# yjtang249/MIPSFusion

Measured on AMD Instinct MI355X. Metric: rays*samples/s per GPU, full optimisation iteration (fwd + bwd + pose+map Adam), 4096 rays x 64 samples, 640x480 RGB-D, higher is better.
Workload: dtype f32; decoder products as 3 x bf16 pieces of each fp32 operand, 6 bf16 MFMAs per product, fp32 accumulate; 1 GPU; BASELINE config 2: FastCaMo-synth apartment_2, 1 active submap per GPU, 4096 rays x 64 samples, hash grid 2^19 x 16 x 2, 620x460 synthetic RGB-D; rays=4096, samples_per_ray=64, hash_size=19, parallelism=single gpu

## Files before the change

### include/mipsf_compact.h

```cpp
#ifndef MIPSF_COMPACT_H
#define MIPSF_COMPACT_H

#include "mipsf.h"

#ifdef __cplusplus
extern "C" {
#endif

#define MIPSF_LIVE_HEADER 16u
#define MIPSF_LIVE_PAD 0xffffffffu
int mipsf_decoder_live_compact(const float* dout, uint32_t M, uint32_t* live_list, float* dfeat, float* dx, int feat_layout,
                               void* stream);

int mipsf_hashgrid_dx_from_jac_list(const float* jac, const float* dout, float* dx, const uint32_t* live_list, uint32_t M,
                                    const mipsf_grid_meta* meta_host, int layout, void* stream);

#ifdef __cplusplus
}
#endif
#endif
```

### mipsfusion_amd/_lib.py

```python
from __future__ import annotations

import ctypes as C
import os
from typing import Optional

import torch

_HERE = os.path.dirname(os.path.abspath(__file__))
LIB_PATH = os.environ.get("MIPSF_LIB") or os.path.join(_HERE, "libmipsf_hip.so")
MAX_LEVELS = 32
FEAT_AOS, FEAT_LEVEL_MAJOR = 0, 1
PREC = {"f32": 0, "f16x3": 1, "f16": 2, "bf16x3": 3, "bf16x6": 4}


class GridMeta(C.Structure):
    _fields_ = [("n_levels", C.c_uint32), ("n_features", C.c_uint32), ("log2_hashmap_size", C.c_uint32),
                ("base_resolution", C.c_uint32), ("per_level_scale", C.c_float),
                ("log2_per_level_scale", C.c_float), ("n_params", C.c_uint32),
                ("offsets", C.c_uint32 * (MAX_LEVELS + 1)), ("resolutions", C.c_uint32 * MAX_LEVELS),
                ("scales", C.c_float * MAX_LEVELS)]


class DecoderWeights(C.Structure):
    _fields_ = [(n, C.c_void_p) for n in ("w_pts0", "b_pts0", "w_pts2", "b_pts2", "w_rgb0", "b_rgb0",
# ... 17 lines not shown
        a = cls()
        a.struct_size = C.sizeof(cls)
        for k, v in kw.items():
            setattr(a, k, v)
        return a
    cls.new = staticmethod(new)
    return cls


_VP, _CU, _CI = C.c_void_p, C.c_uint32, C.c_int
HashgridBwdArgs = _args("HashgridBwdArgs", [("M", _CU), ("x", _VP), ("params", _VP), ("dout", _VP), ("dparams", _VP), ("dx", _VP),
                                            ("scratch", _VP), ("counters", _VP), ("meta", C.POINTER(GridMeta)),
                                            ("feat_layout", _CI), ("flags", _CU)])
DecoderFwd16Args = _args("DecoderFwd16Args", [("M", _CU), ("packed16", _VP), ("feat", _VP), ("x", _VP), ("out", _VP), ("saved", _VP),
                                              ("tile_live_clear", _VP), ("feat_layout", _CI), ("precision", _CI),
                                              ("sdf_only", _CI), ("lean_record", _CI), ("packed16_floats", _CU)])
DecoderChain16Args = _args("DecoderChain16Args", [("M", _CU), ("packed16", _VP), ("x", _VP), ("out", _VP), ("dout", _VP),
                                                  ("saved", _VP), ("dfeat", _VP), ("dx", _VP), ("dact", _VP), ("tile_live", _VP),
                                                  ("feat_layout", _CI), ("flags", _CI), ("packed16_floats", _CU),
                                                  ("live_list", _VP)])
DecoderWgrad16Args = _args("DecoderWgrad16Args", [("M", _CU), ("packed16", _VP), ("feat", _VP), ("x", _VP), ("saved", _VP),
                                                  ("dact", _VP), ("tile_live", _VP), ("grads", C.POINTER(DecoderGrads)),
                                                  ("partial", _VP), ("feat_layout", _CI), ("arithmetic", _CI), ("flags", _CU),
                                                  ("packed16_floats", _CU), ("live_list", _VP)])
RenderFwdArgs = _args("RenderFwdArgs", [("N", _CU), ("S", _CU), ("raw", _VP), ("z_vals", _VP), ("target_rgb", _VP), ("target_d", _VP),
                                        ("counts", _VP), ("cfg", C.POINTER(RenderCfg)), ("rgb", _VP), ("depth", _VP),
                                        ("depth_var", _VP), ("disp", _VP), ("acc", _VP), ("weights", _VP), ("losses", _VP),
                                        ("partial", _VP), ("loss_weights", _VP), ("loss_total", _VP), ("ticket", _VP),
                                        ("sums", _VP), ("draw", _VP)])
RenderBwdArgs = _args("RenderBwdArgs", [("N", _CU), ("S", _CU), ("N_norm", _CU), ("raw", _VP), ("z_vals", _VP), ("target_rgb", _VP),
                                        ("target_d", _VP), ("counts", _VP), ("losses", _VP), ("cfg", C.POINTER(RenderCfg)),
                                        ("g_losses", _VP), ("g_total", _VP), ("loss_weights", _VP), ("g_rgb", _VP),
                                        ("g_depth", _VP), ("draw", _VP), ("flags", _CU)])
RENDER_BWD_KEEP_IF_UNIT = 1

(SIZE_HASHGRID_BWD_SCRATCH, SIZE_HASHGRID_COUNTER_WORDS, SIZE_DECODER_PACKED, SIZE_DECODER_SAVED, SIZE_DECODER_DACT,
 SIZE_DECODER_WGRAD_PARTIAL, SIZE_DECODER_PACKED16, SIZE_DECODER_TILE_WORDS, SIZE_RENDER_PARTIAL, SIZE_PLACE_POSE_SCRATCH,
 SIZE_POSE_RAYS_SCRATCH, SIZE_HASHGRID_DET_SCRATCH, SIZE_DECODER_LIVE_LIST) = range(1, 14)
LIVE_HEADER, LIVE_PAD = 16, 0xFFFFFFFF

HG_DPARAMS_ZERO, HG_ROUTED, HG_DETERMINISTIC = 1, 2, 4
HG_DET_PIECE = 512
HG_DET_MAX_ITEMS = 1 << 31
TILE_ORDER_MAX_M = 1 << 27
WGRAD_LEAN_DACT, WGRAD_DETERMINISTIC = 1, 2


ADAM_MAX_TENSORS = 16


class AdamTensors(C.Structure):
    _fields_ = [("count", C.c_uint32), ("param", C.c_void_p * ADAM_MAX_TENSORS), ("grad", C.c_void_p * ADAM_MAX_TENSORS),
                ("exp_avg", C.c_void_p * ADAM_MAX_TENSORS), ("exp_avg_sq", C.c_void_p * ADAM_MAX_TENSORS),
                ("numel", C.c_uint64 * ADAM_MAX_TENSORS)]


ADAM_MAX_GROUPS = 8
ADAM_SMALL_MAX_NUMEL = 16384


class AdamSmall(C.Structure):
    _fields_ = [("n_groups", C.c_uint32), ("n_tensors", C.c_uint32),
                ("step_dev", C.c_void_p * ADAM_MAX_GROUPS), ("hyper_dev", C.c_void_p * ADAM_MAX_GROUPS),
                ("lr", C.c_float * ADAM_MAX_GROUPS), ("beta1", C.c_float * ADAM_MAX_GROUPS),
                ("beta2", C.c_float * ADAM_MAX_GROUPS), ("eps", C.c_float * ADAM_MAX_GROUPS),
                ("weight_decay", C.c_float * ADAM_MAX_GROUPS),
                ("param", C.c_void_p * ADAM_MAX_TENSORS), ("grad", C.c_void_p * ADAM_MAX_TENSORS),
                ("exp_avg", C.c_void_p * ADAM_MAX_TENSORS), ("exp_avg_sq", C.c_void_p * ADAM_MAX_TENSORS),
                ("numel", C.c_uint32 * ADAM_MAX_TENSORS), ("group_of", C.c_uint32 * ADAM_MAX_TENSORS)]


_P = C.c_void_p
_U32, _U64, _I, _F, _D = C.c_uint32, C.c_uint64, C.c_int, C.c_float, C.c_double

SIGNATURES = {
    "mipsf_last_error": (C.c_char_p, []),
    "mipsf_abi_version": (_I, []),
    "mipsf_device_cu_count": (_I, []),
    "mipsf_buffer_size": (_U64, [_I, _U32, _U32, _U32, C.POINTER(GridMeta)]),
    "mipsf_hashgrid_meta_init": (_I, [C.POINTER(GridMeta), _U32, _U32, _U32, _U32, _D]),
    "mipsf_hashgrid_fwd": (_I, [_P, _P, _P, _P, _U32, C.POINTER(GridMeta), _I, _P]),
    "mipsf_hashgrid_dx_from_jac": (_I, [_P, _P, _P, _P, _U32, C.POINTER(GridMeta), _I, _P]),
    "mipsf_hashgrid_bwd": (_I, [C.POINTER(HashgridBwdArgs), _P]),
    "mipsf_hashgrid_route": (_I, [_P, _P, _U32, C.POINTER(GridMeta), _P]),
    "mipsf_hashgrid_indices": (_I, [_P, _P, _U32, C.POINTER(GridMeta), _P]),
    "mipsf_freq_fwd": (_I, [_P, _P, _U32, _U32, _U32, _P]),
    "mipsf_freq_bwd": (_I, [_P, _P, _P, _U32, _U32, _U32, _P]),
    "mipsf_decoder_pack": (_I, [C.POINTER(DecoderWeights), _P, _P]),
    "mipsf_decoder_pack_host": (_I, [C.POINTER(DecoderWeights), _P]),
    "mipsf_decoder_fwd": (_I, [_P, _P, _I, _P, _P, _I, _P, _P, _U32, _P]),
    "mipsf_decoder_fwd_sdf": (_I, [_P, _P, _I, _P, _P, _I, _P, _U32, _P]),
    "mipsf_decoder_bwd": (_I, [_P, _P, _I, _P, _P, _I, _P, _P, _P, _P, _P, _P, C.POINTER(DecoderGrads), _P, _P,
                               _U32, _P]),
    "mipsf_decoder_bwd_chain": (_I, [_P, _I, _P, _I, _P, _P, _P, _P, _P, _P, _P, _U32, _P]),
    "mipsf_decoder_wgrad": (_I, [_P, _I, _P, _P, _I, _P, _P, C.POINTER(DecoderGrads), _P, _I, _U32, _P]),
    "mipsf_decoder_pack16": (_I, [C.POINTER(DecoderWeights), _P, _I, _P]),
    "mipsf_decoder_fwd16": (_I, [C.POINTER(DecoderFwd16Args), _P]),
    "mipsf_decoder_bwd_chain16": (_I, [C.POINTER(DecoderChain16Args), _P]),
    "mipsf_decoder_wgrad16": (_I, [C.POINTER(DecoderWgrad16Args), _P]),
    "mipsf_sample_rays": (_I, [_P, _P, _P, _P, _P, _P, _P, C.POINTER(RenderCfg), _P, _P, _P, _U32, _P]),
    "mipsf_normalise_points": (_I, [_P, C.POINTER(RenderCfg), _P, _U32, _P]),
    "mipsf_render_fwd": (_I, [C.POINTER(RenderFwdArgs), _P]),
    "mipsf_loss_finalize_sums": (_I, [_P, C.POINTER(RenderCfg), _U32, _U32, _P, _P, _P, _P]),
    "mipsf_render_bwd": (_I, [C.POINTER(RenderBwdArgs), _P]),
    "mipsf_gather_pose_place_fwd": (_I, [_P, _U64, _P, _P, _P, _P, _U32, _U32, _P, _P, _P, _P, _P, C.POINTER(RenderCfg), _P, _P,
                                         _P, _P, _P, _P, _U32, _P]),
    "mipsf_place_pose_bwd": (_I, [_P, _P, C.POINTER(RenderCfg), _P, _U32, _U32, _P, _P, _P, _P, _P, _U32, _U32, _I, _P]),
    "mipsf_rays_bwd": (_I, [_P, _P, C.POINTER(RenderCfg), _P, _P, _U32, _U32, _P]),
    "mipsf_normalise_bwd": (_I, [_P, C.POINTER(RenderCfg), _P, _U32, _P]),
    "mipsf_pose_rays_fwd": (_I, [_P, _U64, _P, _P, _P, _P, _U32, _U32, _P, _P, _P, _P, _P, _P, _U32, _P]),
    "mipsf_pose_handover": (_I, [_P, _I, _P, _P, _P]),
    "mipsf_pose_rays_bwd": (_I, [_P, _P, _P, _U32, _U32, _P, _P, _P, _P, _P, _U32, _I, _P]),
    "mipsf_adam_step": (_I, [_P, _P, _P, _P, _U64, _F, _F, _F, _F, _F, _U32, _P, _I, _P]),
    "mipsf_adam_advance_n": (_I, [_P, _P, _P, _P, _P, _U32, _P]),
    "mipsf_adam_step_multi": (_I, [C.POINTER(AdamTensors), _F, _F, _F, _F, _F, _U32, _P, _I, _P]),
    "mipsf_adam_step_small": (_I, [C.POINTER(AdamSmall), _I, _P]),
    "mipsf_adam_step_all": (_I, [C.POINTER(AdamSmall), _I, _P, _P]),
    "mipsf_ro_fitness": (_I, [_P, _U32, _P, _F, _P, _U32, _U32, _P]),
    "mipsf_ro_fitness_sdf": (_I, [_P, _P, _F, _P, _U32, _U32, _I, _P]),
    "mipsf_ro_particles": (_I, [_P, _P, _P, _P, C.POINTER(RenderCfg), _P, _P, _U32, _U32, _I, _P]),
    "mipsf_ro_update": (_I, [_P, _P, _P, _F, _F, _U32, _P]),
    "mipsf_gather_rays": (_I, [_P, _U64, _P, _U32, _P, _P, _P, _P, _P]),
}


SIZE_MCUBES_OFFSET_WORDS, SIZE_MCUBES_WELD_SLOTS, SIZE_MCUBES_WELD_WORDS = 20, 21, 22
MCUBES_BLOCK_CELLS = 4096
McubesArgs = _args("McubesArgs", [("X", _CU), ("Y", _CU), ("Z", _CU), ("isovalue", C.c_float), ("truncation", C.c_float),
                                  ("volume", _VP), ("cases", _VP), ("block_offsets", _VP), ("soup", _VP), ("cell_ids", _VP),
                                  ("capacity_tris", _CU)])
McubesWeldArgs = _args("McubesWeldArgs", [("T", _CU), ("soup", _VP), ("scratch", _VP), ("vertices", _VP), ("faces", _VP),
                                          ("counts", _VP), ("max_rounds", _CU)])
COMPACT_SIGNATURES = {
    "mipsf_decoder_live_compact": (_I, [_P, _U32, _P, _P, _P, _I, _P]),
    "mipsf_hashgrid_dx_from_jac_list": (_I, [_P, _P, _P, _P, _U32, C.POINTER(GridMeta), _I, _P]),
}

MESH_SIGNATURES = {
    "mipsf_mcubes_count": (_I, [C.POINTER(McubesArgs), _P]),
    "mipsf_mcubes_emit": (_I, [C.POINTER(McubesArgs), _P]),
    "mipsf_mcubes_weld": (_I, [C.POINTER(McubesWeldArgs), _P]),
}


FUSE_KF_FLOATS = 16
FUSE_IN_BOX, FUSE_SEEN = 1, 2


class FusePoints(C.Structure):
    _fields_ = [("points", _VP), ("ticks", _VP * 3), ("dims", _CU * 3), ("lo", _CU * 3), ("size", _CU * 3), ("first", _CU), ("n", _CU)]


class FuseCamera(C.Structure):
    _fields_ = [("fx", C.c_float), ("fy", C.c_float), ("cx", C.c_float), ("cy", C.c_float), ("W", C.c_float), ("H", C.c_float),
                ("edge", C.c_float), ("k", _CU), ("keyframes", _VP)]


FuseVisibilityArgs = _args("FuseVisibilityArgs", [("pts", FusePoints), ("cam", FuseCamera), ("seen", _VP)])
FuseLocalArgs = _args("FuseLocalArgs", [("pts", FusePoints), ("w2l", C.c_float * 12), ("sub", C.c_double * 3), ("div", C.c_double * 3),
                                        ("out", _VP)])
FuseAccumulateArgs = _args("FuseAccumulateArgs", [("pts", FusePoints), ("cam", FuseCamera), ("rows", _VP), ("n_rows", _CU),
                                                  ("channels", _CU), ("sigmoid", _CU), ("values", _VP), ("entropy", _VP),
                                                  ("value_stride", _CU), ("entropy_stride", _CU), ("use_obb", _CU),
                                                  ("obb_centre", C.c_double * 3), ("obb_axes", C.c_double * 9),
                                                  ("obb_half", C.c_double * 3), ("centroid", C.c_float * 3), ("sigma", C.c_float),
                                                  ("gauss_k", C.c_float), ("num", _VP), ("den", _VP), ("flags", _VP)])
FuseFinalizeArgs = _args("FuseFinalizeArgs", [("n", _CU), ("channels", _CU), ("num", _VP), ("den", _VP), ("flags", _VP), ("out", _VP),
                                              ("volume", _VP)])
FuseLabelArgs = _args("FuseLabelArgs", [("F", _CU), ("E", _CU), ("pairs", _VP), ("labels", _VP), ("counts", _VP), ("max_rounds", _CU),
                                        ("resume", _CU)])
FUSE_SIGNATURES = {
    "mipsf_fuse_visibility": (_I, [C.POINTER(FuseVisibilityArgs), _P]),
    "mipsf_fuse_local_points": (_I, [C.POINTER(FuseLocalArgs), _P]),
    "mipsf_fuse_accumulate": (_I, [C.POINTER(FuseAccumulateArgs), _P]),
    "mipsf_fuse_finalize": (_I, [C.POINTER(FuseFinalizeArgs), _P]),
    "mipsf_fuse_label_components": (_I, [C.POINTER(FuseLabelArgs), _P]),
}


ICP_KNN = 30
ICP_RESULT_DOUBLES = 20
ICP_MAX_POINTS, ICP_MAX_CELLS = 1 << 27, 1 << 26
ICP_WS_CLOUD, ICP_WS_GRID, ICP_WS_REGISTER = 1, 2, 3
IcpCloudArgs = _args("IcpCloudArgs", [("n", _CU), ("k", _CU), ("rows_per_owner", _CU), ("rows", _VP), ("owner", _VP), ("poses", _VP),
                                      ("points", _VP), ("count", _VP), ("workspace", _VP)])
IcpBinArgs = _args("IcpBinArgs", [("n", _CU), ("max_cells", _CU), ("points", _VP), ("min_edge", C.c_double), ("grid", _VP)])
IcpNearestArgs = _args("IcpNearestArgs", [("n_source", _CU), ("n_target", _CU), ("max_cells", _CU), ("source", _VP), ("grid", _VP),
                                          ("max_dist", C.c_double), ("partner", _VP), ("d2", _VP)])
IcpNormalsArgs = _args("IcpNormalsArgs", [("n", _CU), ("max_cells", _CU), ("points", _VP), ("grid", _VP), ("normals", _VP),
                                          ("neighbours", _VP)])
IcpRegisterArgs = _args("IcpRegisterArgs", [("n_source", _CU), ("n_target", _CU), ("max_cells", _CU), ("max_iteration", _CU),
                                            ("source", _VP), ("grid", _VP), ("target_normals", _VP), ("max_dist", C.c_double),
                                            ("relative_fitness", C.c_double), ("relative_rmse", C.c_double), ("result", _VP),
                                            ("partner", _VP), ("workspace", _VP)])
ICP_SIGNATURES = {
    "mipsf_icp_workspace_bytes": (_U64, [_I, _U32, _U32]),
    "mipsf_icp_cloud": (_I, [C.POINTER(IcpCloudArgs), _P]),
    "mipsf_icp_bin": (_I, [C.POINTER(IcpBinArgs), _P]),
    "mipsf_icp_nearest": (_I, [C.POINTER(IcpNearestArgs), _P]),
    "mipsf_icp_normals": (_I, [C.POINTER(IcpNormalsArgs), _P]),
    "mipsf_icp_register": (_I, [C.POINTER(IcpRegisterArgs), _P]),
}


POSEGRAPH_MAX_NODES, POSEGRAPH_MAX_EDGES, POSEGRAPH_LDS_NODES, POSEGRAPH_RESULT_DOUBLES = 64, 1024, 20, 8
POSEGRAPH_FACTORISATION_FAILED, POSEGRAPH_NAN_QUALITY, POSEGRAPH_BAD_EDGE = 1, 2, 4
PosegraphArgs = _args("PosegraphArgs", [("n_nodes", _CU), ("n_edges", _CU), ("input_f64", _CU), ("anchors", _VP), ("edges", _VP),
                                        ("observations", _VP), ("weights", _VP), ("steps", _CU), ("patience", _CU),
                                        ("max_rejects", _CU), ("reserved", _CU), ("decreasing", C.c_double), ("radius", C.c_double),
                                        ("min_diag", C.c_double), ("anchors_out", _VP), ("anchors_out32", _VP), ("result", _VP),
                                        ("workspace", _VP)])
POSEGRAPH_SIGNATURES = {
    "mipsf_posegraph_workspace_bytes": (_U64, [_U32, _U32]),
    "mipsf_posegraph_optimize": (_I, [C.POINTER(PosegraphArgs), _P]),
}


SUBMAP_MAX_BOXES, SUBMAP_MAX_TOP_KF, SUBMAP_HEADER_WORDS, SUBMAP_BOX_WORDS, SUBMAP_WORKSPACE_BYTES = 64, 10, 16, 12, 8192
# ... 69 lines not shown
    "mipsf_raster_workspace_bytes": (_U64, [_I, _U32, _U32, _U32, _U32]),
    "mipsf_raster_depth": (_I, [C.POINTER(RasterDepthArgs), _P]),
    "mipsf_raster_l1": (_I, [C.POINTER(RasterL1Args), _P]),
    "mipsf_raster_visible": (_I, [C.POINTER(RasterVisibleArgs), _P]),
}


TSDF_MAX_VOXELS, TSDF_MAX_SIDE, TSDF_VIEW_CHUNK, TSDF_BRICK = 0x7FFFFFFF, 8192, 256, (8, 8, 16)
TSDF_NO_CULL = 1
TSDF_MAX_BRICKS = 0xFFFFFF
TSDF_RECORD_WORDS = 2
TsdfIntegrateArgs = _args("TsdfIntegrateArgs", [("X", _CU), ("Y", _CU), ("Z", _CU), ("n", _CU), ("H", _CU), ("W", _CU), ("flags", _CU),
                                                ("fx", C.c_double), ("fy", C.c_double), ("cx", C.c_double), ("cy", C.c_double),
                                                ("trunc", C.c_double), ("depth_max", C.c_double), ("max_weight", C.c_double),
                                                ("ticks", _VP * 3), ("depth", _VP), ("rgb", _VP), ("poses", _VP), ("tsdf", _VP),
                                                ("weight", _VP), ("color", _VP), ("record", _VP)])
TsdfSampleArgs = _args("TsdfSampleArgs", [("X", _CU), ("Y", _CU), ("Z", _CU), ("m", _CU), ("reserved", _CU), ("points", _VP),
                                          ("weight", _VP), ("color", _VP), ("out", _VP)])
TSDF_SIGNATURES = {
    "mipsf_tsdf_integrate": (_I, [C.POINTER(TsdfIntegrateArgs), _P]),
    "mipsf_tsdf_sample": (_I, [C.POINTER(TsdfSampleArgs), _P]),
}


TRACK_MAX_SAMPLES, TRACK_TILE, TRACK_RESULT_DOUBLES, TRACK_MAX_ITERATION, TRACK_MAX_VIEWS = 0x100000, 16, 20, 1000, 65535
TRACK_NO_SKIP = 1
TRACK_WS_RAYCAST, TRACK_WS_REGISTER = 1, 2
TRACK_RECORD_WORDS = 2
TrackRaycastArgs = _args("TrackRaycastArgs", [("X", _CU), ("Y", _CU), ("Z", _CU), ("n", _CU), ("H", _CU), ("W", _CU), ("flags", _CU),
                                              ("origin", C.c_double * 3), ("voxel", C.c_double), ("trunc", C.c_double),
                                              ("fx", C.c_double), ("fy", C.c_double), ("cx", C.c_double), ("cy", C.c_double),
                                              ("near", C.c_double), ("far", C.c_double), ("step", C.c_double), ("min_weight", C.c_double),
                                              ("tsdf", _VP), ("weight", _VP), ("color", _VP), ("poses", _VP), ("depth", _VP),
                                              ("normals", _VP), ("color_out", _VP), ("record", _VP), ("workspace", _VP)])
TrackRegisterArgs = _args("TrackRegisterArgs", [("H", _CU), ("W", _CU), ("max_iteration", _CU),
                                                ("fx", C.c_double), ("fy", C.c_double), ("cx", C.c_double), ("cy", C.c_double),
                                                ("depth_max", C.c_double), ("max_dist", C.c_double), ("relative_fitness", C.c_double),
                                                ("relative_rmse", C.c_double), ("model_depth", _VP), ("model_normals", _VP),
                                                ("pose_ref", _VP), ("live", _VP), ("pose_init", _VP), ("result", _VP), ("pose_out", _VP),
                                                ("partner", _VP), ("workspace", _VP)])
TRACK_SIGNATURES = {
    "mipsf_track_workspace_bytes": (_U64, [_I, _U32, _U32, _U32]),
    "mipsf_track_raycast": (_I, [C.POINTER(TrackRaycastArgs), _P]),
    "mipsf_track_register": (_I, [C.POINTER(TrackRegisterArgs), _P]),
}


IMAGE_F32, IMAGE_F64 = 0, 1
IMAGE_WINDOW, IMAGE_TILE_H, IMAGE_TILE_W, IMAGE_MAX_CHANNELS, IMAGE_MAX_SIDE = 11, 16, 32, 4, 8192
IMAGE_MAX_PLANES, IMAGE_MAX_VALUES, IMAGE_ERROR_MAX_BLOCKS = 65535, 0x7FFFFFFF, 256
IMAGE_WS_ERROR, IMAGE_WS_SSIM = 1, 2
IMAGE_ERROR_RECORD_BYTES, IMAGE_SSIM_RECORD_BYTES = 32, 32


class ImageErrorRecord(C.Structure):
    _fields_ = [("sum_sq", C.c_double), ("sum_abs", C.c_double), ("max_abs", C.c_double), ("count", C.c_uint64)]


class ImageSsimRecord(C.Structure):
    _fields_ = [("sum_ssim", C.c_double), ("sum_cs", C.c_double), ("count", C.c_uint64), ("reserved", C.c_uint64)]


ImageErrorArgs = _args("ImageErrorArgs", [("n", _CU), ("H", _CU), ("W", _CU), ("C", _CU), ("dtype", _CU), ("a", _VP), ("b", _VP),
                                          ("records", _VP), ("workspace", _VP)])
ImageSsimArgs = _args("ImageSsimArgs", [("n", _CU), ("H", _CU), ("W", _CU), ("C", _CU), ("dtype", _CU), ("window", C.c_double * 11),
                                        ("C1", C.c_double), ("C2", C.c_double), ("a", _VP), ("b", _VP), ("records", _VP),
                                        ("workspace", _VP)])
ImagePool2Args = _args("ImagePool2Args", [("n", _CU), ("H", _CU), ("W", _CU), ("C", _CU), ("dtype", _CU), ("in_", _VP), ("out", _VP)])
IMAGE_SIGNATURES = {
    "mipsf_image_workspace_bytes": (_U64, [_I, _U32, _U32, _U32, _U32]),
    "mipsf_image_error": (_I, [C.POINTER(ImageErrorArgs), _P]),
    "mipsf_image_ssim": (_I, [C.POINTER(ImageSsimArgs), _P]),
    "mipsf_image_pool2": (_I, [C.POINTER(ImagePool2Args), _P]),
}


def buffer_size(which: int, n: int = 0, a: int = 0, b: int = 0, meta=None) -> int:
    v = lib().mipsf_buffer_size(which, n, a, b, C.byref(meta) if meta is not None else None)
    if v == 0xFFFFFFFFFFFFFFFF:
        raise RuntimeError((lib().mipsf_last_error() or b"mipsf_buffer_size: bad query").decode())
    return int(v)


_lib: Optional[C.CDLL] = None


def lib() -> C.CDLL:
    global _lib
    if _lib is None:
        if not os.path.exists(LIB_PATH):
            raise RuntimeError(
                f"{LIB_PATH} is missing: build it with `python -c 'import __graft_entry__ as g; g.build()'` "
                "(or `make -C mipsfusion_amd/csrc`). There is no CPU fallback.")
        handle = C.CDLL(LIB_PATH)
        for name, (res, args) in list(SIGNATURES.items()) + (list(MESH_SIGNATURES.items())
                                       + list(FUSE_SIGNATURES.items()) + list(ICP_SIGNATURES.items())
                                       + list(COMPACT_SIGNATURES.items()) + list(POSEGRAPH_SIGNATURES.items())
                                       + list(SUBMAP_SIGNATURES.items()) + list(EVAL_SIGNATURES.items())
                                       + list(RASTER_SIGNATURES.items()) + list(TSDF_SIGNATURES.items())
                                       + list(IMAGE_SIGNATURES.items()) + list(TRACK_SIGNATURES.items())):
            fn = getattr(handle, name)
            fn.restype = res
            fn.argtypes = args
        if handle.mipsf_abi_version() != 2:
            raise RuntimeError("libmipsf_hip.so ABI version mismatch")
        _lib = handle
    return _lib


KEPT_BLOCK_CACHES = []


def check(rc: int, what: str = "") -> None:
    if rc != 0:
        msg = lib().mipsf_last_error().decode(errors="replace")
        for cache in KEPT_BLOCK_CACHES:
            cache.clear()
        raise RuntimeError(f"libmipsf_hip {what} failed (code {rc}): {msg}")


def stream_ptr() -> int:
    return torch._C._cuda_getCurrentRawStream(torch._C._cuda_getDevice())


def dptr(t: Optional[torch.Tensor], dtype=torch.float32) -> Optional[int]:
    if t is None:
        return None
    if not t.is_cuda:
        raise RuntimeError("mipsfusion_amd operators need GPU tensors (no CPU fallback exists)")
    if t.device.index != torch._C._cuda_getDevice():
        raise RuntimeError(f"tensor lives on cuda:{t.device.index} but the current device is "
                           f"cuda:{torch._C._cuda_getDevice()}; wrap the call in torch.cuda.device(tensor.device)")
    if t.dtype != dtype:
        raise RuntimeError(f"expected {dtype}, got {t.dtype}")
    if not t.is_contiguous():
        raise RuntimeError("tensor must be contiguous")
    return t.data_ptr()


def make_grid_meta(n_levels=16, n_features=2, log2_hashmap_size=19, base_resolution=16,
                   per_level_scale=2.0) -> GridMeta:
    m = GridMeta()
    check(lib().mipsf_hashgrid_meta_init(C.byref(m), n_levels, n_features, log2_hashmap_size, base_resolution,
                                         float(per_level_scale)), "hashgrid_meta_init")
    return m
```

### mipsfusion_amd/csrc/hashgrid.hip

```cpp
#include "common.h"
#include "decoder_layout.h"

namespace mipsf {

constexpr uint32_t P1 = 2654435761u;
constexpr uint32_t P2 = 805459861u;
constexpr int HG_BLOCK = 256;

struct Cell {
    uint32_t c[3];
    float f[3];
};

__device__ __forceinline__ Cell locate(const float* __restrict__ x, uint32_t i, float scale) {
    Cell r;
#pragma unroll
    for (int d = 0; d < 3; ++d) {
        const float pos = fmaf(scale, x[3 * (size_t)i + d], 0.5f);
        const float fl = floorf(pos);
        r.c[d] = (uint32_t)(int)fl;
        r.f[d] = pos - fl;
    }
    return r;
}
// ... 7 lines not shown
            idx -= size;
            if (idx >= size) idx %= size;
        }
        return idx;
    }
    const uint32_t h = cx ^ (cy * P1) ^ (cz * P2);
    return MODE == 1 ? (h & (size - 1u)) : (h % size);
}

__host__ __device__ inline bool level_is_hashed(uint32_t res, uint32_t size) {
    uint64_t stride = 1;
    for (int d = 0; d < 3; ++d) {
        if (stride > size) break;
        stride *= res;
        stride &= 0xFFFFFFFFull;
    }
    return size < stride;
}

__device__ __forceinline__ int decode_level(uint32_t n_levels, uint32_t nchunk, uint32_t& chunk) {
    const uint32_t b = blockIdx.x;
    const uint32_t xcd = b & 7u;
    const uint32_t j = b >> 3;
    const uint32_t slot = j / nchunk;
    chunk = j - slot * nchunk;
    const uint32_t nslots = (n_levels + 7u) / 8u;
    return (int)(xcd + 8u * (nslots - 1u - slot));
}

template <int MODE>
__device__ __forceinline__ void corner_indices_m(const Cell& cell, uint32_t res, uint32_t size, uint32_t idx[8]) {
#pragma unroll
    for (int c = 0; c < 8; ++c) {
        idx[c] = corner_index<MODE>(cell.c[0] + (c & 1), cell.c[1] + ((c >> 1) & 1), cell.c[2] + ((c >> 2) & 1),
                                    res, size);
    }
}

__device__ __forceinline__ int level_mode(uint32_t res, uint32_t size) {
    if (!level_is_hashed(res, size)) return 0;
    return (size & (size - 1u)) == 0u ? 1 : 2;
}

__device__ __forceinline__ void corner_indices(int mode, const Cell& cell, uint32_t res, uint32_t size,
                                               uint32_t idx[8]) {
    if (mode == 0) corner_indices_m<0>(cell, res, size, idx);
    else if (mode == 1) corner_indices_m<1>(cell, res, size, idx);
    else corner_indices_m<2>(cell, res, size, idx);
}

__device__ __forceinline__ void corner_weights(const Cell& cell, float w[8]) {
#pragma unroll
    for (int c = 0; c < 8; ++c) {
        float t = (c & 1) ? cell.f[0] : 1.0f - cell.f[0];
        t = t * ((c & 2) ? cell.f[1] : 1.0f - cell.f[1]);
        t = t * ((c & 4) ? cell.f[2] : 1.0f - cell.f[2]);
        w[c] = t;
    }
}

template <int LAYOUT>
__device__ __forceinline__ size_t feat_index(uint32_t i, uint32_t level, uint32_t M, uint32_t L) {
    return LAYOUT == MIPSF_FEAT_AOS ? ((size_t)i * L + level) * 2 : ((size_t)level * M + i) * 2;
}

__device__ __forceinline__ void level_jacobian(const Cell& cell, const float2 (&v)[8], float scale, int d, float& s0,
                                               float& s1) {
    s0 = 0.f, s1 = 0.f;
#pragma unroll
    for (int sub = 0; sub < 4; ++sub) {
        const int d0 = d == 0 ? 1 : 0;
        const int d1 = d == 2 ? 1 : 2;
        const int b0 = sub & 1, b1 = (sub >> 1) & 1;
        float wgt = scale;
        wgt = wgt * (b0 ? cell.f[d0] : 1.0f - cell.f[d0]);
        wgt = wgt * (b1 ? cell.f[d1] : 1.0f - cell.f[d1]);
        const int left = (b0 << d0) | (b1 << d1);
        const int right = left | (1 << d);
        s0 = s0 + wgt * (v[right].x - v[left].x);
        s1 = s1 + wgt * (v[right].y - v[left].y);
    }
}

template <int LAYOUT, bool JAC>
__global__ __launch_bounds__(HG_BLOCK) void hashgrid_fwd_kernel(const float* __restrict__ x,
                                                                const float2* __restrict__ table,
                                                                float* __restrict__ out, float* __restrict__ jac,
                                                                uint32_t M, GridLevels g, uint32_t nchunk) {
    uint32_t chunk;
    const int level = decode_level(g.n_levels, nchunk, chunk);
    if (level >= (int)g.n_levels) return;
    const uint32_t i = chunk * HG_BLOCK + threadIdx.x;
    if (i >= M) return;

    const uint32_t off = g.offsets[level];
    const uint32_t size = g.offsets[level + 1] - off;
    const uint32_t res = g.res[level];
    const Cell cell = locate(x, i, g.scale[level]);
    uint32_t idx[8];
    corner_indices(level_mode(res, size), cell, res, size, idx);
    float w[8];
    corner_weights(cell, w);
    const float2* lvl = table + off;
    float2 v[8];
#pragma unroll
    for (int c = 0; c < 8; ++c) v[c] = lvl[idx[c]];
    float a0 = 0.f, a1 = 0.f;
#pragma unroll
    for (int c = 0; c < 8; ++c) {
        a0 = fmaf(w[c], v[c].x, a0);
        a1 = fmaf(w[c], v[c].y, a1);
    }
    typedef float f32x2_t __attribute__((ext_vector_type(2)));
    f32x2_t* dst = reinterpret_cast<f32x2_t*>(out + feat_index<LAYOUT>(i, level, M, g.n_levels));
    __builtin_nontemporal_store(f32x2_t{a0, a1}, dst);
    if (JAC) {
        f32x2_t* j2 = reinterpret_cast<f32x2_t*>(jac) + (size_t)level * 3 * M + i;
#pragma unroll
        for (int d = 0; d < 3; ++d) {
            float s0, s1;
            level_jacobian(cell, v, g.scale[level], d, s0, s1);
            __builtin_nontemporal_store(f32x2_t{s0, s1}, j2 + (size_t)d * M);
        }
    }
}

constexpr int SC_BLOCK = 1024;
#ifndef MIPSF_SC_PLANAR
#define MIPSF_SC_PLANAR 1
#endif
#if MIPSF_SC_PLANAR
#define SC_ACC0(e) (e)
#define SC_ACC1(e) (sc_plane1 + (e))
#else
#define SC_ACC0(e) (2 * (e))
#define SC_ACC1(e) (2 * (e) + 1)
#endif
#ifndef MIPSF_RT_BLOCK
#define MIPSF_RT_BLOCK 512
#endif
constexpr int RT_BLOCK = MIPSF_RT_BLOCK;
#ifndef MIPSF_SC_MAX_SLICE
#define MIPSF_SC_MAX_SLICE 8192
#endif
constexpr uint32_t SC_MAX_SLICE = MIPSF_SC_MAX_SLICE;
#ifndef MIPSF_SC_SLICE_LOG2
#define MIPSF_SC_SLICE_LOG2 13
#endif
constexpr uint32_t SC_SLICE_LOG2 = MIPSF_SC_SLICE_LOG2;
#ifndef MIPSF_SC_PART
#define MIPSF_SC_PART 24576
#endif
#ifndef MIPSF_SC_PART_DENSE
#define MIPSF_SC_PART_DENSE 8192
#endif
#ifndef MIPSF_SC_RUN
#define MIPSF_SC_RUN 4
#endif
#ifndef MIPSF_SC_SKIP_ZERO
#define MIPSF_SC_SKIP_ZERO 1
#endif
constexpr uint32_t SC_PART = MIPSF_SC_PART;
constexpr uint32_t SC_PART_DENSE = MIPSF_SC_PART_DENSE;
constexpr uint32_t SC_PART_MIN = SC_PART < SC_PART_DENSE ? SC_PART : SC_PART_DENSE;
constexpr uint32_t SC_RUN = MIPSF_SC_RUN;
constexpr uint32_t SC_ROUTE_UNR = 4;
constexpr uint32_t SC_MAX_NS = 512;
constexpr uint32_t SC_MAX_BINS = 8192;
#ifndef MIPSF_SC_MASKED_MAX_M
#define MIPSF_SC_MASKED_MAX_M (1u << 24)
#endif
constexpr uint32_t SC_MASKED_MAX_M = MIPSF_SC_MASKED_MAX_M;

struct ScatterPlan {
    uint32_t n_levels;
    uint32_t n_slices[MIPSF_MAX_LEVELS];
    uint32_t slice_entries[MIPSF_MAX_LEVELS];
    uint32_t slice_shift[MIPSF_MAX_LEVELS];
    uint32_t bin0[MIPSF_MAX_LEVELS + 1];
    uint32_t n_bins;
    uint32_t max_items;
    uint32_t max_slice;
    uint32_t dense_bins;
    uint32_t fresh;
    uint32_t w_count, w_first, w_parts, w_nitems, w_items;
    uint64_t w_records, w_partial, w_end;
};

static ScatterPlan make_plan(const GridLevels& g, uint32_t M) {
    ScatterPlan p = {};
    p.n_levels = g.n_levels;
    uint32_t bins = 0;
    for (uint32_t l = 0; l < g.n_levels; ++l) {
        const uint32_t size = g.offsets[l + 1] - g.offsets[l];
        const bool one = size <= SC_MAX_SLICE;
        const uint32_t ns = one ? 1u : (size + (1u << SC_SLICE_LOG2) - 1) >> SC_SLICE_LOG2;
        p.n_slices[l] = ns;
        p.slice_entries[l] = one ? size : (1u << SC_SLICE_LOG2);
        p.slice_shift[l] = one ? 31u : SC_SLICE_LOG2;
        p.bin0[l] = bins;
        bins += ns;
    }
    p.bin0[g.n_levels] = bins;
    p.n_bins = bins;
    for (uint32_t l = 0; l < g.n_levels; ++l) {
        if (level_is_hashed(g.res[l], g.offsets[l + 1] - g.offsets[l])) break;
        p.dense_bins = p.bin0[l + 1];
    }
    for (uint32_t l = 0; l < g.n_levels; ++l) p.max_slice = p.slice_entries[l] > p.max_slice ? p.slice_entries[l] : p.max_slice;
    const uint64_t max_records = 8ull * g.n_levels * M;
    p.max_items = (uint32_t)((max_records + SC_PART_MIN - 1) / SC_PART_MIN) + bins;
    uint64_t w = 0;
    p.w_count = (uint32_t)w, w += bins;
    p.w_nitems = (uint32_t)w, w += 4;
    p.w_first = (uint32_t)w, w += bins;
    p.w_parts = (uint32_t)w, w += bins;
    w = (w + 3) / 4 * 4;
    p.w_items = (uint32_t)w;
    w = (w + 15) / 16 * 16;
    p.w_records = w, w += (uint64_t)bins * M;
    w = (w + 15) / 16 * 16;
    p.w_partial = w, w += (uint64_t)p.max_items * SC_MAX_SLICE * 2;
    p.w_end = w;
    return p;
}

__global__ void scatter_zero_kernel(uint32_t* __restrict__ ws, uint32_t n) {
    const uint32_t i = blockIdx.x * blockDim.x + threadIdx.x;
    if (i < n) ws[i] = 0u;
}

__device__ __forceinline__ uint32_t ranked_add(uint32_t* cnt, uint32_t s, bool active, bool aggregate) {
    if (!aggregate) return active ? atomicAdd(&cnt[s], 1u) : 0u;
    const uint32_t lane = threadIdx.x & 63u;
    uint32_t rank = 0;
    unsigned long long todo = __ballot(active);
    while (todo) {
        const int leader = __ffsll((long long)todo) - 1;
        const uint32_t s0 = (uint32_t)__shfl((int)s, leader, 64);
        const unsigned long long m = __ballot(active && s == s0);
        uint32_t b = 0;
        if ((int)lane == leader) b = atomicAdd(&cnt[s0], (uint32_t)__popcll(m));
        b = (uint32_t)__shfl((int)b, leader, 64);
        if (active && s == s0) rank = b + (uint32_t)__popcll(m & ((1ull << lane) - 1ull));
        todo &= ~m;
    }
    return rank;
}

__device__ __forceinline__ void route_groups_general(int mode, const Cell& cell, uint32_t res, uint32_t size,
                                                     uint32_t shift, uint32_t (&s)[8], uint32_t (&m)[8]) {
    uint32_t idx[8];
    corner_indices(mode, cell, res, size, idx);
#pragma unroll
    for (int c = 0; c < 8; ++c) s[c] = idx[c] >> shift;
#pragma unroll
    for (int c = 0; c < 8; ++c) {
        bool first = true;
        uint32_t mm = 0;
#pragma unroll
        for (int k = 0; k < 8; ++k) {
            if (k < c) first = first && (s[k] != s[c]);
            mm |= (s[k] == s[c]) ? (1u << k) : 0u;
        }
        m[c] = first ? mm : 0u;
    }
}

__device__ __forceinline__ bool route_groups_dense(const Cell& cell, uint32_t res, uint32_t size, uint32_t shift,
                                                   uint32_t (&s)[8], uint32_t (&m)[8]) {
    uint32_t idx[8];
    corner_indices_m<0>(cell, res, size, idx);
    const uint32_t lo = idx[0] >> shift, hi = idx[7] >> shift;
    uint32_t m_lo = 0, m_hi = 0;
#pragma unroll
    for (int c = 0; c < 8; ++c) {
        const uint32_t q = idx[c] >> shift;
        m_lo |= (q == lo) ? (1u << c) : 0u;
        m_hi |= (q == hi) ? (1u << c) : 0u;
    }
    s[0] = lo, m[0] = m_lo;
    s[1] = hi, m[1] = hi != lo ? m_hi : 0u;
    return (m_lo | m_hi) == 0xffu;
}

__device__ __forceinline__ bool route_groups_hashed_pow2(const Cell& cell, uint32_t size, uint32_t shift,
                                                         uint32_t (&s)[8], uint32_t (&m)[8]) {
#pragma unroll
    for (int p = 0; p < 4; ++p) {
        const uint32_t cy = cell.c[1] + (p & 1), cz = cell.c[2] + (p >> 1);
        s[p] = ((cell.c[0] ^ (cy * P1) ^ (cz * P2)) & (size - 1u)) >> shift;
        m[p] = 3u << (2 * p);
    }
#pragma unroll
    for (int p = 1; p < 4; ++p)
#pragma unroll
        for (int q = 0; q < p; ++q) {
// ... 174 lines not shown
        mp[u][1] = m[4] | (m[5] << 8) | (m[6] << 16) | (m[7] << 24);
    }
    RT_MARK(3);
    __syncthreads();
    RT_MARK(4);
    for (uint32_t q = threadIdx.x; q < ns; q += RT_BLOCK)
        base[q] = cnt[q] ? atomicAdd(&cw[plan.w_count + bin0 + q], cnt[q]) : 0u;
    if (MIPSF_SC_STAGE && threadIdx.x < 64) {
        constexpr uint32_t PER = SC_MAX_NS / 64;
        uint32_t c[PER], sum = 0;
#pragma unroll
        for (uint32_t q2 = 0; q2 < PER; ++q2) {
            const uint32_t q = threadIdx.x * PER + q2;
            c[q2] = q < ns ? cnt[q] : 0u;
            sum += c[q2];
        }
        uint32_t incl = sum;
#pragma unroll
        for (int d = 1; d < 64; d <<= 1) {
            const uint32_t v = (uint32_t)__shfl_up((int)incl, d, 64);
            incl += (int)threadIdx.x >= d ? v : 0u;
        }
        uint32_t run = incl - sum;
#pragma unroll
        for (uint32_t q2 = 0; q2 < PER; ++q2) {
            const uint32_t q = threadIdx.x * PER + q2;
            if (q < ns) lstart[q] = run;
            run += c[q2];
        }
    }
    RT_MARK(5);
    __syncthreads();
    RT_MARK(6);
#pragma unroll
    for (uint32_t u = 0; u < SC_ROUTE_UNR; ++u) {
        const uint32_t i = mine[u];
#pragma unroll
        for (int q = 0; q < 8; ++q) {
            if (q == 4 && !__any(mp[u][1] != 0u)) break;
            const uint32_t m = (mp[u][q >> 2] >> (8 * (q & 3))) & 0xffu;
            if (m) {
                const uint32_t sl = (sp[u][q >> 1] >> (16 * (q & 1))) & 0xffffu;
                const uint32_t rk = (rp[u][q >> 1] >> (16 * (q & 1))) & 0xffffu;
                if (MIPSF_SC_STAGE) {
                    const uint32_t p = lstart[sl] + rk;
                    if (p < STAGE_CAP) {
                        stage[p] = masked ? (i | (m << 24)) : i;
                        continue;
                    }
                }
                rec[(size_t)(bin0 + sl) * M + base[sl] + rk] = masked ? (i | (m << 24)) : i;
            }
        }
    }
    RT_MARK(7);
    if (MIPSF_SC_STAGE) {
        __syncthreads();
        RT_MARK(8);
        const uint32_t wave = threadIdx.x >> 6, lane = threadIdx.x & 63u;
        for (uint32_t q = wave; q < ns; q += RT_BLOCK / 64) {
            const uint32_t n = cnt[q], src = lstart[q];
            uint32_t* dstp = rec + (size_t)(bin0 + q) * M + base[q];
            for (uint32_t p = lane; p < n && src + p < STAGE_CAP; p += 64) dstp[p] = stage[src + p];
        }
    }
#ifdef MIPSF_RT_TRACE
    RT_MARK(9);
    for (int q = 2; q < 9; ++q) tr_acc[q] += tr_t[q + 1] - tr_t[q];
    ++tr_levels;
#endif
    }
#ifdef MIPSF_RT_TRACE
    if ((threadIdx.x & 63u) == 0u) {
        unsigned long long* tr = reinterpret_cast<unsigned long long*>(ws + plan.w_end + 64) + (size_t)(blockIdx.x * (RT_BLOCK / 64) + (threadIdx.x >> 6)) * 10;
        for (int q = 0; q < 9; ++q) tr[q] = tr_acc[q];
        tr[9] = (unsigned long long)(group | (tr_levels << 8));
    }
#endif
}
__device__ __forceinline__ uint32_t part_of(const ScatterPlan& plan, uint32_t bin) {
    return bin < plan.dense_bins ? SC_PART_DENSE : SC_PART;
}

template <int LAYOUT>
__device__ __forceinline__ void scatter_item(const float* __restrict__ x, const float* __restrict__ dout,
                                             float* __restrict__ dparams, uint32_t M, const GridLevels& g,
                                             const ScatterPlan& plan, uint32_t* __restrict__ ws, double* __restrict__ acc,
                                             const uint4 desc, const uint32_t item_index) {
    const uint32_t item = desc.x;
    const uint32_t sc_plane1 = plan.max_slice;
    (void)sc_plane1;
    const uint32_t bin = item & 0xffffu, part = item >> 16;
    const bool single = desc.z == 1u;
    uint32_t level = 0;
    while (level + 1 < plan.n_levels && bin >= plan.bin0[level + 1]) ++level;
    const uint32_t slice = bin - plan.bin0[level];
    const uint32_t off = g.offsets[level];
    const uint32_t size = g.offsets[level + 1] - off;
    const uint32_t se = plan.slice_entries[level];
    const uint32_t begin = slice * se;
    const uint32_t count = begin + se <= size ? se : size - begin;
    const uint32_t res = g.res[level];
    const float scale = g.scale[level];
    const uint32_t n_rec_bin = desc.y;
    const uint32_t r0 = part * part_of(plan, bin);
    const uint32_t n_rec = n_rec_bin - r0 < part_of(plan, bin) ? n_rec_bin - r0 : part_of(plan, bin);
    const uint32_t* __restrict__ rec = ws + plan.w_records + (size_t)bin * M + r0;

    {
#if MIPSF_SC_PLANAR
        for (uint32_t e = threadIdx.x; e < count; e += SC_BLOCK) acc[SC_ACC0(e)] = 0.0, acc[SC_ACC1(e)] = 0.0;
#else
        double2* z = reinterpret_cast<double2*>(acc);
        for (uint32_t e = threadIdx.x; e < count; e += SC_BLOCK) z[e] = make_double2(0.0, 0.0);
#endif
    }
    float2* dst = reinterpret_cast<float2*>(dparams) + off + begin;
    constexpr uint32_t FL = SC_MAX_SLICE / SC_BLOCK;
    float2 cur[FL];
    if (single && !plan.fresh) {
#pragma unroll
        for (uint32_t k = 0; k < FL; ++k) {
            const uint32_t e = threadIdx.x + k * SC_BLOCK;
            cur[k] = e < count ? dst[e] : make_float2(0.f, 0.f);
        }
    }
    __syncthreads();

    const int mode = level_mode(res, size);
    const bool masked = M <= SC_MASKED_MAX_M;
    uint32_t cc[3] = {0u, 0u, 0u};
    float sum[8][2];
    bool open = false;
    auto flush = [&]() {
#ifdef MIPSF_SC_ABL_DENSE_NOATOM
        if (mode == 0) { asm volatile("" :: "v"(sum[0][0]), "v"(sum[7][1])); return; }
#endif
        Cell cell;
        cell.c[0] = cc[0], cell.c[1] = cc[1], cell.c[2] = cc[2];
        uint32_t idx[8];
        corner_indices(mode, cell, res, size, idx);
        uint32_t hit = 0;
#pragma unroll
        for (int c = 0; c < 8; ++c) {
            idx[c] -= begin;
            hit |= (idx[c] < count) ? (1u << c) : 0u;
        }
        if (mode == 0) {
#pragma unroll
            for (int c = 0; c < 8; ++c) {
                if (hit >> c & 1u) {
                    atomicAdd(&acc[SC_ACC0(idx[c])], (double)sum[c][0]);
                    atomicAdd(&acc[SC_ACC1(idx[c])], (double)sum[c][1]);
                }
            }
            return;
        }
        while (hit) {
            const int c = __ffs((int)hit) - 1;
            hit &= hit - 1u;
            uint32_t e = idx[0];
            float v0 = sum[0][0], v1 = sum[0][1];
#pragma unroll
            for (int k = 1; k < 8; ++k) {
                e = (c == k) ? idx[k] : e;
                v0 = (c == k) ? sum[k][0] : v0;
                v1 = (c == k) ? sum[k][1] : v1;
            }
            atomicAdd(&acc[SC_ACC0(e)], (double)v0);
            atomicAdd(&acc[SC_ACC1(e)], (double)v1);
// ... 70 lines not shown
                    const uint32_t cx = cell.c[0] + (c & 1), cy = cell.c[1] + ((c >> 1) & 1), cz = cell.c[2] + ((c >> 2) & 1);
                    const uint32_t e = (mode == 1 ? corner_index<1>(cx, cy, cz, res, size) : corner_index<2>(cx, cy, cz, res, size)) - begin;
                    float wgt = (c & 1) ? cell.f[0] : 1.0f - cell.f[0];
                    wgt = wgt * ((c & 2) ? cell.f[1] : 1.0f - cell.f[1]);
                    wgt = wgt * ((c & 4) ? cell.f[2] : 1.0f - cell.f[2]);
                    atomicAdd(&acc[SC_ACC0(e)], (double)(wgt * gy.x));
                    atomicAdd(&acc[SC_ACC1(e)], (double)(wgt * gy.y));
                }
            }
        }
    } else {
    constexpr int UNR = (int)SC_RUN;
    const uint32_t chunk_id = threadIdx.x;
    for (uint32_t r = chunk_id * SC_RUN; r < n_rec; r += SC_BLOCK * SC_RUN) {
        const uint32_t re = r + SC_RUN < n_rec ? r + SC_RUN : n_rec;
        uint32_t si[UNR];
        float px[UNR][3];
        float2 pg[UNR];
#pragma unroll
        for (int u = 0; u < UNR; ++u) {
            si[u] = rec[r + u < re ? r + u : re - 1];
            si[u] = masked ? (si[u] & 0xffffffu) : si[u];
        }
#pragma unroll
        for (int u = 0; u < UNR; ++u) {
            const uint32_t ii = si[u];
#ifdef MIPSF_SC_ABL_DENSE_NOGATHER
            px[u][0] = (float)(ii & 4095u) * (1.0f / 4096.0f), px[u][1] = (float)((ii >> 6) & 4095u) * (1.0f / 4096.0f);
            px[u][2] = (float)((ii >> 12) & 63u) * (1.0f / 64.0f);
            pg[u] = make_float2(1e-3f, 2e-3f);
#else
            px[u][0] = x[3 * (size_t)ii], px[u][1] = x[3 * (size_t)ii + 1], px[u][2] = x[3 * (size_t)ii + 2];
            pg[u] = *reinterpret_cast<const float2*>(dout + feat_index<LAYOUT>(ii, level, M, g.n_levels));
#endif
        }
#pragma unroll
        for (int u = 0; u < UNR; ++u) {
            if (r + u >= re) break;
            Cell cell;
#pragma unroll
            for (int d = 0; d < 3; ++d) {
                const float pos = fmaf(scale, px[u][d], 0.5f);
                const float fl = floorf(pos);
                cell.c[d] = (uint32_t)(int)fl;
                cell.f[d] = pos - fl;
            }
            const bool same = open && cell.c[0] == cc[0] && cell.c[1] == cc[1] && cell.c[2] == cc[2];
            if (!same) {
#ifndef MIPSF_SC_ABL_DENSE_NOMID
                if (open) flush();
#endif
                cc[0] = cell.c[0], cc[1] = cell.c[1], cc[2] = cell.c[2];
#pragma unroll
                for (int c = 0; c < 8; ++c) sum[c][0] = 0.0f, sum[c][1] = 0.0f;
                open = true;
            }
            const float2 gy = pg[u];
#pragma unroll
            for (int c = 0; c < 8; ++c) {
                float wgt = (c & 1) ? cell.f[0] : 1.0f - cell.f[0];
                wgt = wgt * ((c & 2) ? cell.f[1] : 1.0f - cell.f[1]);
                wgt = wgt * ((c & 4) ? cell.f[2] : 1.0f - cell.f[2]);
                sum[c][0] = sum[c][0] + wgt * gy.x;
                sum[c][1] = sum[c][1] + wgt * gy.y;
            }
        }
        if (open) flush();
        open = false;
    }
    }
    __syncthreads();

    auto a2 = [&](uint32_t e) { return make_double2(acc[SC_ACC0(e)], acc[SC_ACC1(e)]); };
    if (single) {
#pragma unroll
        for (uint32_t k = 0; k < FL; ++k) {
            const uint32_t e = threadIdx.x + k * SC_BLOCK;
            if (e < count) {
                const double2 a = a2(e);
                dst[e] = plan.fresh ? make_float2((float)a.x, (float)a.y) : make_float2(cur[k].x + (float)a.x, cur[k].y + (float)a.y);
            }
        }
    } else {
        float2* pdst = reinterpret_cast<float2*>(reinterpret_cast<float*>(ws) + plan.w_partial) +
                       (size_t)item_index * SC_MAX_SLICE;
        for (uint32_t e = threadIdx.x; e < count; e += SC_BLOCK) {
            const double2 a = a2(e);
            pdst[e] = make_float2((float)a.x, (float)a.y);
        }
    }
}


template <int LAYOUT>
__global__ __launch_bounds__(SC_BLOCK) void hashgrid_scatter_persist_kernel(const float* __restrict__ x,
                                                                           const float* __restrict__ dout,
                                                                           float* __restrict__ dparams, uint32_t M,
                                                                           GridLevels g, ScatterPlan plan,
                                                                           uint32_t* __restrict__ ws,
                                                                           uint32_t* __restrict__ cw) {
    extern __shared__ __attribute__((aligned(16))) double acc[];
    __shared__ uint32_t wtot[16];
    __shared__ uint32_t sh_total, sh_next;
    __shared__ uint4 sh_desc;
    constexpr uint32_t PER = SC_MAX_BINS / SC_BLOCK;
    const uint32_t t = threadIdx.x;
    uint32_t* scnt = reinterpret_cast<uint32_t*>(acc + 2 * (size_t)plan.max_slice);
    uint32_t litm = 0;
#pragma unroll
    for (uint32_t k = 0; k < PER; ++k) {
        const uint32_t b = t * PER + k;
        const uint32_t c = b < plan.n_bins ? cw[plan.w_count + b] : 0u;
        if (b < plan.n_bins) scnt[b] = c;
        litm += (c + part_of(plan, b) - 1) / part_of(plan, b);
    }
    uint32_t oitm;
    {
        uint32_t incl = litm;
#pragma unroll
        for (int d = 1; d < 64; d <<= 1) {
            const uint32_t v = (uint32_t)__shfl_up((int)incl, d, 64);
            incl += (int)(t & 63u) >= d ? v : 0u;
        }
        if ((t & 63u) == 63u) wtot[t >> 6] = incl;
        __syncthreads();
        uint32_t before = 0;
        for (uint32_t q = 0; q < (t >> 6); ++q) before += wtot[q];
        oitm = before + incl - litm;
        if (t == SC_BLOCK - 1) sh_total = before + incl;
    }
    {
        uint32_t first = oitm;
        for (uint32_t k = 0; k < PER; ++k) {
            const uint32_t b = t * PER + k;
            if (b >= plan.n_bins) break;
            const uint32_t parts = (scnt[b] + part_of(plan, b) - 1) / part_of(plan, b);
            cw[plan.w_first + b] = first, cw[plan.w_parts + b] = parts;
            first += parts;
        }
    }
    __syncthreads();
    const uint32_t total = sh_total;
    if (t == 0) sh_next = __hip_atomic_fetch_add(&cw[plan.w_nitems + 1], 1u, __ATOMIC_RELAXED, __HIP_MEMORY_SCOPE_AGENT);
    __syncthreads();
    if (sh_next == gridDim.x - 1) {
        for (uint32_t b = t; b < plan.n_bins; b += SC_BLOCK) cw[plan.w_count + b] = 0u;
    }
    for (;;) {
        __syncthreads();
        if (t == 0) sh_next = __hip_atomic_fetch_add(&cw[plan.w_nitems], 1u, __ATOMIC_RELAXED, __HIP_MEMORY_SCOPE_AGENT);
        __syncthreads();
        const uint32_t i = sh_next;
        if (i >= total) break;
        if (i >= oitm && i < oitm + litm) {
            uint32_t first = oitm;
            for (uint32_t k = 0; k < PER; ++k) {
                const uint32_t b = t * PER + k;
                if (b >= plan.n_bins) break;
                const uint32_t c = scnt[b];
                const uint32_t parts = (c + part_of(plan, b) - 1) / part_of(plan, b);
                if (i >= first && i < first + parts) sh_desc = make_uint4(b | ((i - first) << 16), c, parts, 0u);
                first += parts;
            }
        }
        __syncthreads();
        const uint4 desc = sh_desc;
#ifdef MIPSF_SC_TRACE
        const uint64_t tr_t0 = wall_clock64();
#endif
        scatter_item<LAYOUT>(x, dout, dparams, M, g, plan, ws, acc, desc, i);
#ifdef MIPSF_SC_TRACE
        __syncthreads();
        if (t == 0) {
            const uint64_t tr_t1 = wall_clock64();
            uint32_t* tr = ws + plan.w_end + 64 + 8 * (size_t)i;
            tr[0] = i, tr[1] = desc.x, tr[2] = desc.y, tr[3] = (uint32_t)tr_t0, tr[4] = (uint32_t)tr_t1;
            tr[5] = __builtin_amdgcn_s_getreg((31 << 11) | 20), tr[6] = blockIdx.x, tr[7] = desc.z;
            if (i == 0) ws[plan.w_end + 63] = total;
        }
#endif
    }
    __syncthreads();
    if (t == 0) {
        if (__hip_atomic_fetch_add(&cw[plan.w_nitems + 2], 1u, __ATOMIC_RELAXED, __HIP_MEMORY_SCOPE_AGENT) == gridDim.x - 1) {
            __hip_atomic_store(&cw[plan.w_nitems], 0u, __ATOMIC_RELAXED, __HIP_MEMORY_SCOPE_AGENT);
            __hip_atomic_store(&cw[plan.w_nitems + 1], 0u, __ATOMIC_RELAXED, __HIP_MEMORY_SCOPE_AGENT);
            __hip_atomic_store(&cw[plan.w_nitems + 2], 0u, __ATOMIC_RELAXED, __HIP_MEMORY_SCOPE_AGENT);
        }
    }
}

__global__ __launch_bounds__(256) void hashgrid_scatter_reduce_kernel(float* __restrict__ dparams, GridLevels g,
                                                                      ScatterPlan plan, const uint32_t* __restrict__ ws,
                                                                      const uint32_t* __restrict__ cw) {
    const uint32_t bin = blockIdx.x;
    const uint32_t parts = cw[plan.w_parts + bin];
    if (parts <= 1) return;
    uint32_t level = 0;
    while (level + 1 < plan.n_levels && bin >= plan.bin0[level + 1]) ++level;
    const uint32_t size = g.offsets[level + 1] - g.offsets[level];
    const uint32_t se = plan.slice_entries[level];
    const uint32_t begin = (bin - plan.bin0[level]) * se;
    const uint32_t count = begin + se <= size ? se : size - begin;
    const uint32_t e = blockIdx.y * 256 + threadIdx.x;
    if (e >= count) return;
    const float2* p2 = reinterpret_cast<const float2*>(reinterpret_cast<const float*>(ws) + plan.w_partial) +
                       (size_t)cw[plan.w_first + bin] * SC_MAX_SLICE + e;
    float2* d = reinterpret_cast<float2*>(dparams) + g.offsets[level] + begin + e;
    float2 cur = plan.fresh ? make_float2(0.f, 0.f) : *d;
    float2 a = make_float2(0.f, 0.f);
    for (uint32_t q = 0; q < parts; q += 8) {
        float2 v[8];
#pragma unroll
        for (uint32_t k = 0; k < 8; ++k) v[k] = q + k < parts ? p2[(size_t)(q + k) * SC_MAX_SLICE] : make_float2(0.f, 0.f);
#pragma unroll
        for (uint32_t k = 0; k < 8; ++k) a.x += v[k].x, a.y += v[k].y;
    }
    cur.x += a.x, cur.y += a.y;
    *d = cur;
}

template <int LAYOUT>
MIPSF_SINGLE_FP32 __global__ __launch_bounds__(HG_BLOCK) void hashgrid_dx_kernel(const float* __restrict__ x,
                                                               const float2* __restrict__ table,
                                                               const float* __restrict__ dout,
                                                               float* __restrict__ dxl, uint32_t M, GridLevels g,
                                                               uint32_t nchunk) {
    uint32_t chunk;
    const int level = decode_level(g.n_levels, nchunk, chunk);
    if (level >= (int)g.n_levels) return;
    const uint32_t i = chunk * HG_BLOCK + threadIdx.x;
    if (i >= M) return;
    const uint32_t off = g.offsets[level];
    const uint32_t size = g.offsets[level + 1] - off;
    const uint32_t res = g.res[level];
    const float scale = g.scale[level];
    const Cell cell = locate(x, i, scale);
    uint32_t idx[8];
    corner_indices(level_mode(res, size), cell, res, size, idx);
    const float2 gy = *reinterpret_cast<const float2*>(dout + feat_index<LAYOUT>(i, level, M, g.n_levels));
    const float2* lvl = table + off;
    float2 v[8];
#pragma unroll
    for (int c = 0; c < 8; ++c) v[c] = lvl[idx[c]];
    float gx[3];
#pragma unroll
    for (int d = 0; d < 3; ++d) {
        float s0, s1;
        level_jacobian(cell, v, scale, d, s0, s1);
        gx[d] = s0 * gy.x + s1 * gy.y;
    }
    float* o = dxl + ((size_t)level * M + i) * 3;
    o[0] = gx[0], o[1] = gx[1], o[2] = gx[2];
}

__global__ __launch_bounds__(256) void hashgrid_dx_reduce_kernel(const float* __restrict__ dxl, float* __restrict__ dx,
                                                                 uint64_t n3, uint32_t L) {
    const uint64_t t = (uint64_t)blockIdx.x * blockDim.x + threadIdx.x;
    if (t >= n3) return;
    float a = 0.f;
    for (uint32_t l = 0; l < L; ++l) a += dxl[(uint64_t)l * n3 + t];
    dx[t] += a;
}

template <int LAYOUT>
MIPSF_SINGLE_FP32 __global__ __launch_bounds__(256) void hashgrid_dx_jac_kernel(const float* __restrict__ jac,
                                                              const float* __restrict__ dout, float* __restrict__ dx,
                                                              uint32_t M, uint32_t L,
                                                              const uint32_t* __restrict__ tiles,
                                                              const uint32_t* __restrict__ live_list) {
    uint32_t i = blockIdx.x * blockDim.x + threadIdx.x;
    if (live_list != nullptr) {
        if (i >= M || i >= live_list[0]) return;
        i = live_list[MIPSF_LIVE_HEADER + i];
    }
    if (tiles != nullptr) {
        const uint32_t k = i >> 5, cap = mipsf::dl::tl_cap((M + 31u) / 32u);
        uint32_t q = 0, first = 0, total = 0;
#pragma unroll
        for (uint32_t j = 0; j < 8; ++j) {
            const uint32_t n = tiles[64 * j + 32];
            if (k >= total && n != 0u) q = j, first = total;
            total += n;
        }
        if (k >= total) return;
        i = tiles[mipsf::dl::TL_HEADER + q * cap + (k - first)] * 32u + (i & 31u);
    }
    if (i >= M) return;
    float a[3] = {0.f, 0.f, 0.f};
    for (uint32_t l = 0; l < L; ++l) {
        const float2* j2 = reinterpret_cast<const float2*>(jac) + (size_t)l * 3 * M + i;
        const float2 gy = *reinterpret_cast<const float2*>(dout + feat_index<LAYOUT>(i, l, M, L));
#pragma unroll
        for (int d = 0; d < 3; ++d) {
            const float2 j = j2[(size_t)d * M];
            a[d] += j.x * gy.x + j.y * gy.y;
        }
    }
    dx[3 * (size_t)i] += a[0], dx[3 * (size_t)i + 1] += a[1], dx[3 * (size_t)i + 2] += a[2];
}

__global__ __launch_bounds__(HG_BLOCK) void hashgrid_indices_kernel(const float* __restrict__ x,
                                                                    uint32_t* __restrict__ out, uint32_t M,
                                                                    GridLevels g, uint32_t nchunk) {
    uint32_t chunk;
    const int level = decode_level(g.n_levels, nchunk, chunk);
    if (level >= (int)g.n_levels) return;
    const uint32_t i = chunk * HG_BLOCK + threadIdx.x;
    if (i >= M) return;
    const uint32_t size = g.offsets[level + 1] - g.offsets[level];
    const uint32_t res = g.res[level];
    const Cell cell = locate(x, i, g.scale[level]);
    uint32_t idx[8];
    corner_indices(level_mode(res, size), cell, res, size, idx);
#pragma unroll
    for (int c = 0; c < 8; ++c) out[((size_t)i * g.n_levels + level) * 8 + c] = idx[c];
}

static int to_levels(const mipsf_grid_meta* m, GridLevels& g) {
    MIPSF_REQUIRE(m != nullptr, "meta is null");
    MIPSF_REQUIRE(m->n_features == 2, "only n_features_per_level == 2 is built");
    MIPSF_REQUIRE(m->n_levels >= 1 && m->n_levels <= MIPSF_MAX_LEVELS, "bad n_levels");
    g.n_levels = m->n_levels;
    for (uint32_t l = 0; l <= m->n_levels; ++l) g.offsets[l] = m->offsets[l];
    for (uint32_t l = 0; l < m->n_levels; ++l) {
        g.res[l] = m->resolutions[l];
        g.scale[l] = m->scales[l];
    }
    return 0;
}

static inline uint32_t grid_blocks(uint32_t M, uint32_t L, uint32_t& nchunk) {
    nchunk = (M + HG_BLOCK - 1) / HG_BLOCK;
    return 8u * ((L + 7u) / 8u) * nchunk;
}

constexpr uint32_t DET_BLOCK = 256;
constexpr uint32_t DET_PER_THREAD = 16;
constexpr uint32_t DET_TILE = DET_BLOCK * DET_PER_THREAD;
constexpr uint32_t DET_PIECE = MIPSF_HG_DET_PIECE;
static_assert((DET_PIECE & (DET_PIECE - 1u)) == 0u, "the piece length is a power of two");

template <int LAYOUT>
__global__ __launch_bounds__(DET_BLOCK) void det_emit_kernel(const float* __restrict__ x, const float* __restrict__ dout,
                                                             uint32_t* __restrict__ keys, uint32_t M, GridLevels g,
                                                             uint32_t dead) {
    const uint32_t level = blockIdx.y;
    const uint32_t i = blockIdx.x * DET_BLOCK + threadIdx.x;
    if (i >= M) return;
    const float2 gy = *reinterpret_cast<const float2*>(dout + feat_index<LAYOUT>(i, level, M, g.n_levels));
    uint32_t k[8];
    if (gy.x == 0.f && gy.y == 0.f) {
#pragma unroll
        for (int c = 0; c < 8; ++c) k[c] = dead;
    } else {
        const uint32_t off = g.offsets[level];
        const uint32_t size = g.offsets[level + 1] - off;
        const uint32_t res = g.res[level];
        const Cell cell = locate(x, i, g.scale[level]);
        corner_indices(level_mode(res, size), cell, res, size, k);
#pragma unroll
        for (int c = 0; c < 8; ++c) k[c] += off;
    }
    uint4* dst = reinterpret_cast<uint4*>(keys + ((size_t)level * M + i) * 8);
    dst[0] = make_uint4(k[0], k[1], k[2], k[3]);
    dst[1] = make_uint4(k[4], k[5], k[6], k[7]);
}

__device__ __forceinline__ uint32_t det_block_scan(uint32_t v, uint32_t* s) {
    s[threadIdx.x] = v;
    __syncthreads();
// ... 192 lines not shown
    p.o_dxl = (o + 15) / 16 * 16;
    p.w_end = p.o_dxl;
    return p;
}

uint64_t hashgrid_det_scratch_floats(const mipsf_grid_meta* meta, uint32_t M, int need_dx) {
    GridLevels g;
    if (to_levels(meta, g)) return 0;
    const DetPlan p = det_plan(g, M);
    return p.w_end + (need_dx ? (uint64_t)g.n_levels * M * 3 : 0) + 64;
}

static int hashgrid_bwd_det(const float* x, const float* params, const float* dout, float* dparams, float* dx, float* scratch,
                            uint32_t M, const mipsf_grid_meta* meta, int layout, bool fresh, void* stream) {
    GridLevels g;
    if (int rc = to_levels(meta, g)) return rc;
    if (M == 0) return 0;
    MIPSF_REQUIRE(x && params && dout && scratch, "null pointer");
    MIPSF_REQUIRE(dparams || dx, "nothing to compute: dparams and dx are both null");
    MIPSF_REQUIRE(layout == MIPSF_FEAT_AOS || layout == MIPSF_FEAT_LEVEL_MAJOR, "bad layout %d", layout);
    MIPSF_REQUIRE(8ull * g.n_levels * M <= MIPSF_HG_DET_MAX_ITEMS,
                  "deterministic scatter: 8 x %u levels x M = %u is above its limit of 2^31 items (M <= %u)", g.n_levels, M,
                  (unsigned)(MIPSF_HG_DET_MAX_ITEMS / (8ull * g.n_levels)));
    const DetPlan p = det_plan(g, M);
    hipStream_t s = (hipStream_t)stream;
    uint32_t* ws = reinterpret_cast<uint32_t*>(scratch);
    if (dparams) {
        const uint32_t n = (uint32_t)p.n, nb = p.nb;
        uint32_t *keys[2] = {ws + p.o_keys[0], ws + p.o_keys[1]}, *vals[2] = {ws + p.o_vals[0], ws + p.o_vals[1]};
        uint32_t *cnt = ws + p.o_cnt, *tot = ws + p.o_tot, *start = ws + p.o_start;
        double2* psum = reinterpret_cast<double2*>(scratch);
        const dim3 eg((M + DET_BLOCK - 1) / DET_BLOCK, g.n_levels);
        if (layout == MIPSF_FEAT_AOS)
            hipLaunchKernelGGL(det_emit_kernel<MIPSF_FEAT_AOS>, eg, dim3(DET_BLOCK), 0, s, x, dout, keys[0], M, g, p.dead);
        else
            hipLaunchKernelGGL(det_emit_kernel<MIPSF_FEAT_LEVEL_MAJOR>, eg, dim3(DET_BLOCK), 0, s, x, dout, keys[0], M, g, p.dead);
        if (int e = check_launch("hashgrid_det_emit")) return e;
        for (uint32_t pass = 0; pass < p.passes; ++pass) {
            const uint32_t a = pass & 1u, shift = 8u * pass;
            hipLaunchKernelGGL(det_count_kernel, dim3(nb), dim3(DET_BLOCK), 0, s, keys[a], cnt, n, nb, shift);
            hipLaunchKernelGGL(det_scan_kernel, dim3(256), dim3(DET_BLOCK), 0, s, cnt, tot, nb);
            hipLaunchKernelGGL(det_place_kernel, dim3(nb), dim3(DET_BLOCK), 0, s, keys[a], pass ? vals[a] : nullptr, keys[a ^ 1u],
                               vals[a ^ 1u], cnt, tot, n, nb, shift);
            if (int e = check_launch("hashgrid_det_sort")) return e;
        }
        const uint32_t* sk = keys[p.passes & 1u];
        const uint32_t* sv = vals[p.passes & 1u];
        const uint32_t tb = (uint32_t)((p.n + DET_BLOCK - 1) / DET_BLOCK);
        hipLaunchKernelGGL(det_start_kernel, dim3(tb), dim3(DET_BLOCK), 0, s, sk, start, n, p.dead);
#define DET_SUMS(LAY)                                                                                                    \
    do {                                                                                                                 \
        hipLaunchKernelGGL(det_pieces_kernel<LAY>, dim3(tb), dim3(DET_BLOCK), 0, s, x, dout, sk, sv, start, psum, n, M, g, \
                           p.dead);                                                                                      \
        hipLaunchKernelGGL(det_total_kernel<LAY>, dim3(tb), dim3(DET_BLOCK), 0, s, x, dout, sk, sv, psum, dparams, n, M, g, \
                           p.dead, fresh ? 1u : 0u);                                                                     \
    } while (0)
        if (layout == MIPSF_FEAT_AOS) DET_SUMS(MIPSF_FEAT_AOS); else DET_SUMS(MIPSF_FEAT_LEVEL_MAJOR);
#undef DET_SUMS
        if (int e = check_launch("hashgrid_det_sums")) return e;
    }
    if (dx) {
        float* dxl = scratch + p.o_dxl;
        uint32_t nchunk;
        const uint32_t nb = grid_blocks(M, g.n_levels, nchunk);
        const float2* table = reinterpret_cast<const float2*>(params);
        if (layout == MIPSF_FEAT_AOS)
            hipLaunchKernelGGL(hashgrid_dx_kernel<MIPSF_FEAT_AOS>, dim3(nb), dim3(HG_BLOCK), 0, s, x, table, dout, dxl, M, g, nchunk);
        else
            hipLaunchKernelGGL(hashgrid_dx_kernel<MIPSF_FEAT_LEVEL_MAJOR>, dim3(nb), dim3(HG_BLOCK), 0, s, x, table, dout, dxl, M, g, nchunk);
        if (int e = check_launch("hashgrid_dx")) return e;
        const uint64_t n3 = (uint64_t)M * 3;
        hipLaunchKernelGGL(hashgrid_dx_reduce_kernel, dim3((uint32_t)((n3 + 255) / 256)), dim3(256), 0, s, dxl, dx, n3, g.n_levels);
        if (int e = check_launch("hashgrid_dx_reduce")) return e;
    }
    return 0;
}

}

using namespace mipsf;

extern "C" {

static int hashgrid_fwd_impl(const float* x, const float* params, float* out, float* jac, uint32_t M,
                             const mipsf_grid_meta* meta, int layout, void* stream) {
    GridLevels g;
    if (int rc = to_levels(meta, g)) return rc;
    if (M == 0) return 0;
    MIPSF_REQUIRE(x && params && out, "null pointer");
    MIPSF_REQUIRE(layout == MIPSF_FEAT_AOS || layout == MIPSF_FEAT_LEVEL_MAJOR, "bad layout %d", layout);
    uint32_t nchunk;
    const uint32_t nb = grid_blocks(M, g.n_levels, nchunk);
    hipStream_t s = (hipStream_t)stream;
    const float2* table = reinterpret_cast<const float2*>(params);
#define FWD(LAY, J) hipLaunchKernelGGL((hashgrid_fwd_kernel<LAY, J>), dim3(nb), dim3(HG_BLOCK), 0, s, x, table, out, jac, M, g, nchunk)
    if (layout == MIPSF_FEAT_AOS) { if (jac) FWD(MIPSF_FEAT_AOS, true); else FWD(MIPSF_FEAT_AOS, false); }
    else { if (jac) FWD(MIPSF_FEAT_LEVEL_MAJOR, true); else FWD(MIPSF_FEAT_LEVEL_MAJOR, false); }
#undef FWD
    return check_launch("hashgrid_fwd");
}

int mipsf_hashgrid_fwd(const float* x, const float* params, float* out, float* jac, uint32_t M,
                       const mipsf_grid_meta* meta, int layout, void* stream) {
    return hashgrid_fwd_impl(x, params, out, jac, M, meta, layout, stream);
}

static int dx_from_jac(const float* jac, const float* dout, float* dx, const uint32_t* tile_live, const uint32_t* live_list, uint32_t M,
                       const mipsf_grid_meta* meta, int layout, void* stream) {
    GridLevels g;
    if (int rc = to_levels(meta, g)) return rc;
    if (M == 0) return 0;
    MIPSF_REQUIRE(jac && dout && dx, "null pointer");
    MIPSF_REQUIRE(layout == MIPSF_FEAT_AOS || layout == MIPSF_FEAT_LEVEL_MAJOR, "bad layout %d", layout);
    hipStream_t s = (hipStream_t)stream;
    if (layout == MIPSF_FEAT_AOS)
        hipLaunchKernelGGL(hashgrid_dx_jac_kernel<MIPSF_FEAT_AOS>, dim3((M + 255) / 256), dim3(256), 0, s, jac, dout, dx, M, g.n_levels, tile_live, live_list);
    else
        hipLaunchKernelGGL(hashgrid_dx_jac_kernel<MIPSF_FEAT_LEVEL_MAJOR>, dim3((M + 255) / 256), dim3(256), 0, s, jac, dout, dx, M, g.n_levels, tile_live, live_list);
    return check_launch("hashgrid_dx_from_jac");
}
int mipsf_hashgrid_dx_from_jac(const float* jac, const float* dout, float* dx, const uint32_t* tile_live, uint32_t M,
                               const mipsf_grid_meta* meta, int layout, void* stream) {
    return dx_from_jac(jac, dout, dx, tile_live, nullptr, M, meta, layout, stream);
}
int mipsf_hashgrid_dx_from_jac_list(const float* jac, const float* dout, float* dx, const uint32_t* live_list, uint32_t M,
                                    const mipsf_grid_meta* meta, int layout, void* stream) {
    MIPSF_REQUIRE(live_list != nullptr, "null live_list");
    return dx_from_jac(jac, dout, dx, nullptr, live_list, M, meta, layout, stream);
}

}
namespace mipsf {
uint64_t hashgrid_bwd_scratch_floats(const mipsf_grid_meta* meta, uint32_t M, int need_dx) {
    GridLevels g;
    if (to_levels(meta, g)) return 0;
    const ScatterPlan p = make_plan(g, M);
#ifdef MIPSF_SC_TRACE
    return p.w_end + 64 + 8ull * p.max_items + 64;
#endif
#ifdef MIPSF_RT_TRACE
    return p.w_end + 64 + 20ull * (RT_BLOCK / 64) * (route_groups(g.n_levels) * ((M + RT_BLOCK * SC_ROUTE_UNR - 1) / (RT_BLOCK * SC_ROUTE_UNR))) + 64;
#endif
    return p.w_end + (need_dx ? (uint64_t)g.n_levels * M * 3 : 0) + 64;
}
uint64_t hashgrid_counter_words(const mipsf_grid_meta* meta) {
    GridLevels g;
    if (to_levels(meta, g)) return 0;
    return make_plan(g, 1).w_items;
}
}
extern "C" {

#ifdef MIPSF_SC_TRACE
uint64_t mipsf_hashgrid_trace_words(const mipsf_grid_meta* meta, uint32_t M, uint32_t* n_rows, uint32_t* bin0) {
    GridLevels g;
    if (to_levels(meta, g)) return 0;
    const ScatterPlan p = make_plan(g, M);
    *n_rows = p.max_items;
    for (uint32_t l = 0; l <= g.n_levels; ++l) bin0[l] = p.bin0[l];
    return p.w_end + 64;
}
#endif


#ifdef MIPSF_RT_TRACE
uint64_t mipsf_hashgrid_rt_trace_words(const mipsf_grid_meta* meta, uint32_t M, uint32_t* n_rows) {
    GridLevels g;
    if (to_levels(meta, g)) return 0;
    const ScatterPlan p = make_plan(g, M);
    *n_rows = (RT_BLOCK / 64) * route_groups(g.n_levels) * ((M + RT_BLOCK * SC_ROUTE_UNR - 1) / (RT_BLOCK * SC_ROUTE_UNR));
    return p.w_end + 64;
}
#endif

static int check_plan(const ScatterPlan& plan, const GridLevels& g, uint32_t M) {
    MIPSF_REQUIRE(plan.n_bins <= SC_MAX_BINS && plan.n_bins <= 0xffffu, "grid too large: %u table slices", plan.n_bins);
    for (uint32_t l = 0; l < g.n_levels; ++l)
        MIPSF_REQUIRE(plan.n_slices[l] <= SC_MAX_NS, "level %u too large: %u slices", l, plan.n_slices[l]);
    MIPSF_REQUIRE(plan.w_end < (1ull << 32), "batch too large for 32-bit scratch offsets (M = %u)", M);
    MIPSF_REQUIRE(((uint64_t)M + SC_PART_MIN - 1) / SC_PART_MIN < (1u << 16), "batch too large (M = %u)", M);
    return 0;
}

static int launch_route(const float* x, const float* dout, int layout, uint32_t* ws, uint32_t* cw, bool clear, uint32_t M,
                        const GridLevels& g, const ScatterPlan& plan, hipStream_t s) {
    if (clear) {
        const uint32_t nz = plan.w_nitems + 4;
        hipLaunchKernelGGL(scatter_zero_kernel, dim3((nz + 255) / 256), dim3(256), 0, s, cw, nz);
    }
    const uint32_t rb = route_groups(g.n_levels) * ((M + RT_BLOCK * SC_ROUTE_UNR - 1) / (RT_BLOCK * SC_ROUTE_UNR));
    if (layout == MIPSF_FEAT_AOS)
        hipLaunchKernelGGL(scatter_route_kernel<MIPSF_FEAT_AOS>, dim3(rb), dim3(RT_BLOCK), 0, s, x, dout, M, g, plan, ws, cw);
    else
        hipLaunchKernelGGL(scatter_route_kernel<MIPSF_FEAT_LEVEL_MAJOR>, dim3(rb), dim3(RT_BLOCK), 0, s, x, dout, M, g, plan, ws, cw);
    return check_launch("hashgrid_route");
}

int mipsf_hashgrid_route(const float* x, float* scratch, uint32_t M, const mipsf_grid_meta* meta, void* stream) {
    GridLevels g;
    if (int rc = to_levels(meta, g)) return rc;
    if (M == 0) return 0;
    MIPSF_REQUIRE(x && scratch, "null pointer");
    const ScatterPlan plan = make_plan(g, M);
    if (int rc = check_plan(plan, g, M)) return rc;
    uint32_t* ws = reinterpret_cast<uint32_t*>(scratch);
    return launch_route(x, nullptr, MIPSF_FEAT_AOS, ws, ws, true, M, g, plan, (hipStream_t)stream);
}

static int hashgrid_bwd_impl(const float* x, const float* params, const float* dout, float* dparams, float* dx,
                             float* scratch, uint32_t* counters, uint32_t M, const mipsf_grid_meta* meta, int layout,
                             bool routed, void* stream, bool fresh = false) {
    GridLevels g;
    if (int rc = to_levels(meta, g)) return rc;
    if (M == 0) return 0;
    MIPSF_REQUIRE(x && params && dout && scratch, "null pointer");
    MIPSF_REQUIRE(dparams || dx, "nothing to compute: dparams and dx are both null");
    MIPSF_REQUIRE(layout == MIPSF_FEAT_AOS || layout == MIPSF_FEAT_LEVEL_MAJOR, "bad layout %d", layout);
    hipStream_t s = (hipStream_t)stream;
    ScatterPlan plan = make_plan(g, M);
    plan.fresh = fresh ? 1u : 0u;
    if (int rc = check_plan(plan, g, M)) return rc;
    uint32_t* ws = reinterpret_cast<uint32_t*>(scratch);
    uint32_t* cw = counters ? counters : ws;
    float* dxl = scratch + ((plan.w_end + 15) / 16) * 16;
    if (dparams) {
        if (!routed)
            if (int e = launch_route(x, MIPSF_SC_SKIP_ZERO ? dout : nullptr, layout, ws, cw, counters == nullptr, M, g, plan, s)) return e;
        const uint32_t lds_bytes = plan.max_slice * 16 + plan.n_bins * 4;
        const int cus = device_cus();
        if (cus <= 0) return 3;
        uint32_t per_cu = (160u * 1024u) / (lds_bytes + 256u);
        per_cu = per_cu < 1u ? 1u : (per_cu > 2048u / SC_BLOCK ? 2048u / SC_BLOCK : per_cu);
        const uint32_t want = (uint32_t)cus * per_cu;
        const uint32_t blocks = plan.max_items < want ? plan.max_items : want;
#define SCATTER(LAY)                                                                                             \
    do {                                                                                                         \
        static uint32_t attr_bytes_dev[MAX_DEVICES] = {0};                                                       \
        uint32_t& attr_bytes = attr_bytes_dev[device_slot()];                                                    \
        if (lds_bytes > attr_bytes) {                                                                            \
            if (hipFuncSetAttribute((const void*)hashgrid_scatter_persist_kernel<LAY>,                           \
                                    hipFuncAttributeMaxDynamicSharedMemorySize, lds_bytes) != hipSuccess) {      \
                set_error("cannot raise dynamic LDS to %u bytes", lds_bytes);                                    \
                return 4;                                                                                        \
            }                                                                                                    \
            attr_bytes = lds_bytes;                                                                              \
        }                                                                                                        \
        hipLaunchKernelGGL((hashgrid_scatter_persist_kernel<LAY>), dim3(blocks), dim3(SC_BLOCK), lds_bytes, s,   \
                           x, dout, dparams, M, g, plan, ws, cw);                                                \
    } while (0)
        if (layout == MIPSF_FEAT_AOS) SCATTER(MIPSF_FEAT_AOS); else SCATTER(MIPSF_FEAT_LEVEL_MAJOR);
#undef SCATTER
        if (int e = check_launch("hashgrid_scatter")) return e;
        hipLaunchKernelGGL(hashgrid_scatter_reduce_kernel, dim3(plan.n_bins, (plan.max_slice + 255) / 256), dim3(256), 0, s,
                           dparams, g, plan, ws, cw);
        if (int e = check_launch("hashgrid_scatter_reduce")) return e;
    }
    if (dx) {
        uint32_t nchunk;
        const uint32_t nb = grid_blocks(M, g.n_levels, nchunk);
        const float2* table = reinterpret_cast<const float2*>(params);
        if (layout == MIPSF_FEAT_AOS)
            hipLaunchKernelGGL(hashgrid_dx_kernel<MIPSF_FEAT_AOS>, dim3(nb), dim3(HG_BLOCK), 0, s, x, table, dout, dxl, M, g, nchunk);
        else
            hipLaunchKernelGGL(hashgrid_dx_kernel<MIPSF_FEAT_LEVEL_MAJOR>, dim3(nb), dim3(HG_BLOCK), 0, s, x, table, dout, dxl, M, g, nchunk);
        if (int e = check_launch("hashgrid_dx")) return e;
        const uint64_t n3 = (uint64_t)M * 3;
        hipLaunchKernelGGL(hashgrid_dx_reduce_kernel, dim3((uint32_t)((n3 + 255) / 256)), dim3(256), 0, s, dxl, dx, n3, g.n_levels);
        if (int e = check_launch("hashgrid_dx_reduce")) return e;
    }
    return 0;
}

int mipsf_hashgrid_bwd(const mipsf_hashgrid_bwd_args* a, void* stream) {
    MIPSF_REQUIRE(a != nullptr, "null argument block");
    MIPSF_REQUIRE(a->struct_size == sizeof(mipsf_hashgrid_bwd_args), "mipsf_hashgrid_bwd_args: struct_size %u, this library expects %u",
                  a->struct_size, (unsigned)sizeof(mipsf_hashgrid_bwd_args));
    MIPSF_REQUIRE((a->flags & ~(uint32_t)(MIPSF_HG_DPARAMS_ZERO | MIPSF_HG_ROUTED | MIPSF_HG_DETERMINISTIC)) == 0u,
                  "unknown flags 0x%x", a->flags);
    if (a->flags & MIPSF_HG_DETERMINISTIC) {
        MIPSF_REQUIRE(!(a->flags & MIPSF_HG_ROUTED), "MIPSF_HG_DETERMINISTIC with MIPSF_HG_ROUTED: the routed scratch belongs to "
                      "the fast scatter; the deterministic path takes its own scratch (MIPSF_SIZE_HASHGRID_DET_SCRATCH)");
        return hashgrid_bwd_det(a->x, a->params, a->dout, a->dparams, a->dx, a->scratch, a->M, a->meta, a->feat_layout,
                                (a->flags & MIPSF_HG_DPARAMS_ZERO) != 0u, stream);
    }
    return hashgrid_bwd_impl(a->x, a->params, a->dout, a->dparams, a->dx, a->scratch, a->counters, a->M, a->meta, a->feat_layout,
                             (a->flags & MIPSF_HG_ROUTED) != 0u, stream, (a->flags & MIPSF_HG_DPARAMS_ZERO) != 0u);
}

int mipsf_hashgrid_indices(const float* x, uint32_t* idx, uint32_t M, const mipsf_grid_meta* meta, void* stream) {
    GridLevels g;
    if (int rc = to_levels(meta, g)) return rc;
    if (M == 0) return 0;
    MIPSF_REQUIRE(x && idx, "null pointer");
    uint32_t nchunk;
    const uint32_t nb = grid_blocks(M, g.n_levels, nchunk);
    hipLaunchKernelGGL(hashgrid_indices_kernel, dim3(nb), dim3(HG_BLOCK), 0, (hipStream_t)stream, x, idx, M, g,
                       nchunk);
    return check_launch("hashgrid_indices");
}

}
```

### mipsfusion_amd/csrc/render.hip

```cpp
#include "pose_dev.h"
#include "render_dev.h"
#include <cstring>
#include <cstddef>

namespace mipsf {

constexpr int RAYS_PER_BLOCK = 4;
constexpr int MAX_S = 256;

struct PlaceCfg {
    uint32_t n_uniform, n_near;
    int perturb;
    float trunc_total;
};

__device__ __forceinline__ void place_ray(const float (&o)[3], const float (&dv)[3], float d, bool has_target,
                                          const float* __restrict__ noise, const float* __restrict__ z_near_off,
                                          const float* __restrict__ z_near_nodepth, const PlaceCfg& pc, const NormCfg& nc,
                                          float* __restrict__ z_vals, float* __restrict__ xn, uint32_t* __restrict__ counts,
                                          float* row, float* rb, const float* sa, uint32_t n, uint32_t lane) {
    const uint32_t nu = pc.n_uniform, nn = pc.n_near, S = nu + nn;
    const bool has_depth = d > 0.f;
    for (uint32_t j = lane; j < nn; j += MIPSF_WAVE) rb[j] = has_depth ? z_near_off[j] + d : z_near_nodepth[j];
    __builtin_amdgcn_fence(__ATOMIC_RELEASE, "wavefront");
// ... 2 lines not shown

    for (uint32_t e = lane; e < S; e += MIPSF_WAVE) {
        float val;
        uint32_t lo = 0, hi;
        if (e < nu) {
            val = sa[e];
            hi = nn;
            while (lo < hi) {
                const uint32_t mid = (lo + hi) >> 1;
                if (rb[mid] < val) lo = mid + 1; else hi = mid;
            }
            row[e + lo] = val;
        } else {
            const uint32_t j = e - nu;
            val = rb[j];
            hi = nu;
            while (lo < hi) {
                const uint32_t mid = (lo + hi) >> 1;
                if (sa[mid] <= val) lo = mid + 1; else hi = mid;
            }
            row[j + lo] = val;
        }
    }
    __builtin_amdgcn_fence(__ATOMIC_RELEASE, "wavefront");
    __builtin_amdgcn_wave_barrier();
    __builtin_amdgcn_fence(__ATOMIC_ACQUIRE, "wavefront");

    uint32_t n_front = 0, n_band = 0;
    for (uint32_t k = lane; k < S; k += MIPSF_WAVE) {
        float z = row[k];
        if (pc.perturb) {
            const float lo = k > 0 ? 0.5f * (z + row[k - 1]) : z;
            const float hi = k + 1 < S ? 0.5f * (row[k + 1] + z) : z;
            z = lo + (hi - lo) * noise[(size_t)n * S + k];
        }
        z_vals[(size_t)n * S + k] = z;
        const float px = o[0] + dv[0] * z, py = o[1] + dv[1] * z, pz = o[2] + dv[2] * z;
        float* out = xn + ((size_t)n * S + k) * 3;
        out[0] = normalise1(px, nc.sub[0], nc.div[0], nc.norm_factor);
        out[1] = normalise1(py, nc.sub[1], nc.div[1], nc.norm_factor);
        out[2] = normalise1(pz, nc.sub[2], nc.div[2], nc.norm_factor);
        if (has_target) {
            const bool front = z < d - pc.trunc_total;
            const bool back = z > d + pc.trunc_total;
            n_front += front ? 1u : 0u;
            n_band += (!front && !back && has_depth) ? 1u : 0u;
        }
    }
    if (has_target && counts) {
        const float f = wave_sum((float)n_front), b = wave_sum((float)n_band);
        if (lane == 0) {
            counts[2 * n] = (uint32_t)f;
            counts[2 * n + 1] = (uint32_t)b;
        }
    }
}

__global__ __launch_bounds__(RAYS_PER_BLOCK * MIPSF_WAVE) void sample_rays_kernel(
    const float* __restrict__ rays_o, const float* __restrict__ rays_d, const float* __restrict__ target_d,
    const float* __restrict__ noise, const float* __restrict__ z_uniform, const float* __restrict__ z_near_off,
    const float* __restrict__ z_near_nodepth, PlaceCfg pc, NormCfg nc, float* __restrict__ z_vals,
    float* __restrict__ xn, uint32_t* __restrict__ counts, uint32_t N) {
    __shared__ float zs[RAYS_PER_BLOCK][MAX_S];
    __shared__ float sb[RAYS_PER_BLOCK][MAX_S];
    __shared__ float sa[MAX_S];
    const uint32_t w = threadIdx.x / MIPSF_WAVE, lane = threadIdx.x & (MIPSF_WAVE - 1);
    const uint32_t n = blockIdx.x * RAYS_PER_BLOCK + w;
    for (uint32_t e = threadIdx.x; e < pc.n_uniform; e += RAYS_PER_BLOCK * MIPSF_WAVE) sa[e] = z_uniform[e];
    __syncthreads();
    if (n >= N) return;
    const float d = target_d ? target_d[n] : 0.f;
    const float o[3] = {rays_o[3 * n], rays_o[3 * n + 1], rays_o[3 * n + 2]};
    const float dv[3] = {rays_d[3 * n], rays_d[3 * n + 1], rays_d[3 * n + 2]};
    place_ray(o, dv, d, target_d != nullptr, noise, z_near_off, z_near_nodepth, pc, nc, z_vals, xn, counts, zs[w], sb[w], sa, n,
              lane);
}

MIPSF_SINGLE_FP32 __global__ __launch_bounds__(RAYS_PER_BLOCK * MIPSF_WAVE) void gather_pose_place_kernel(
    const float* __restrict__ db, uint64_t n_rows, const int64_t* __restrict__ idx, const float* __restrict__ fixed,
    const float* __restrict__ rot, const float* __restrict__ trans, int F, int K, const int64_t* __restrict__ owner,
    const float* __restrict__ noise, const float* __restrict__ z_uniform, const float* __restrict__ z_near_off,
    const float* __restrict__ z_near_nodepth, PlaceCfg pc, NormCfg nc, float* __restrict__ d_cam, float* __restrict__ rgb,
    float* __restrict__ depth, float* __restrict__ z_vals, float* __restrict__ xn, uint32_t* __restrict__ counts,
    uint32_t N) {
    __shared__ float zs[RAYS_PER_BLOCK][MAX_S];
    __shared__ float sb[RAYS_PER_BLOCK][MAX_S];
    __shared__ float sa[MAX_S];
    const uint32_t w = threadIdx.x / MIPSF_WAVE, lane = threadIdx.x & (MIPSF_WAVE - 1);
    const uint32_t n = blockIdx.x * RAYS_PER_BLOCK + w;
    for (uint32_t e = threadIdx.x; e < pc.n_uniform; e += RAYS_PER_BLOCK * MIPSF_WAVE) sa[e] = z_uniform[e];
    __syncthreads();
    if (n >= N) return;
    int64_t r = idx[n];
    if (r < 0) r += (int64_t)n_rows;
    const bool row_ok = r >= 0 && (uint64_t)r < n_rows;
    const float* src = db + 7 * (size_t)(row_ok ? r : 0);
    float v[7];
#pragma unroll
    for (int k = 0; k < 7; ++k) v[k] = row_ok ? src[k] : __builtin_nanf("");
    if (lane == 0) {
        d_cam[3 * (size_t)n] = v[0], d_cam[3 * (size_t)n + 1] = v[1], d_cam[3 * (size_t)n + 2] = v[2];
        rgb[3 * (size_t)n] = v[3], rgb[3 * (size_t)n + 1] = v[4], rgb[3 * (size_t)n + 2] = v[5];
        depth[n] = v[6];
    }
    int64_t p = owner[n];
    if (p < 0) p += F + K;
    const bool in_range = p >= 0 && p < F + K;
    const Mat34 m = load_pose(fixed, rot, trans, F, in_range ? (int)p : 0);
    const float dx = in_range ? v[0] : __builtin_nanf(""), dy = v[1], dz = v[2];
    float o[3], dv[3];
#pragma unroll
    for (int j = 0; j < 3; ++j) {
        dv[j] = (dx * m.r[3 * j] + dy * m.r[3 * j + 1]) + dz * m.r[3 * j + 2];
        o[j] = m.t[j];
    }
    place_ray(o, dv, v[6], true, noise, z_near_off, z_near_nodepth, pc, nc, z_vals, xn, counts, zs[w], sb[w], sa, n, lane);
}

struct LossFinalize {
    const uint32_t* counts;
    uint32_t* ticket;
    float* losses;
    const float* loss_weights;
    float* loss_total;
    double* sums_out;
};

template <bool TRAIN, bool FUSED>
__device__ __forceinline__ void render_fwd_ray(
    const float* __restrict__ raw, const float* __restrict__ z_vals, const float* __restrict__ target_rgb,
    const float* __restrict__ target_d, const RenderCfg& rc, float* __restrict__ rgb_out, float* __restrict__ depth_out,
    float* __restrict__ var_out, float* __restrict__ disp_out, float* __restrict__ acc_out,
    float* __restrict__ weights_out, float* __restrict__ partial, uint32_t N, uint32_t S, float* srow, uint32_t n,
    uint32_t lane, float (&row)[7]) {
    const float* rraw = raw + (size_t)n * S * 10;
    const float* rz = z_vals + (size_t)n * S;
    for (uint32_t k = lane; k < S; k += MIPSF_WAVE) srow[k] = rraw[k * 10 + 3];
    wave_lds_handover();
    const uint32_t kc = first_crossing(srow, S, lane);
    const float z_min = rz[kc];
    const float z_cut = z_min + rc.band;

    float usum = 0.f;
    for (uint32_t k = lane; k < S; k += MIPSF_WAVE) usum += sample_weight(srow[k], rz[k], rc.trunc, z_cut).kept();
    usum = wave_sum(usum);
    const float inv = 1.0f / (usum + 1e-8f);

    float a_r = 0.f, a_g = 0.f, a_b = 0.f, a_d = 0.f, a_w = 0.f;
    for (uint32_t k = lane; k < S; k += MIPSF_WAVE) {
        const float wn = sample_weight(srow[k], rz[k], rc.trunc, z_cut).kept() * inv;
        if (weights_out) weights_out[(size_t)n * S + k] = wn;
        a_r += wn * sigmoidf_(rraw[k * 10 + 0]);
        a_g += wn * sigmoidf_(rraw[k * 10 + 1]);
        a_b += wn * sigmoidf_(rraw[k * 10 + 2]);
        a_d += wn * rz[k];
        a_w += wn;
    }
    a_r = wave_sum(a_r), a_g = wave_sum(a_g), a_b = wave_sum(a_b), a_d = wave_sum(a_d), a_w = wave_sum(a_w);
    float a_v = 0.f;
    for (uint32_t k = lane; k < S; k += MIPSF_WAVE) {
        const float t = rz[k] - a_d;
        a_v += (sample_weight(srow[k], rz[k], rc.trunc, z_cut).kept() * inv) * (t * t);
    }
    a_v = wave_sum(a_v);
    if (lane == 0) store_ray_outputs(n, a_r, a_g, a_b, a_d, a_v, a_w, rgb_out, depth_out, var_out, disp_out, acc_out);
    if (!TRAIN) return;

    const float d = target_d[n];
    float p[4] = {0.f, 0.f, 0.f, 0.f};
    for (uint32_t k = lane; k < S; k += MIPSF_WAVE) loss_terms_add(rz[k], srow[k], d, rc.trunc_total, rc.emd_w, rraw + k * 10 + 5, p);
#pragma unroll
    for (int j = 0; j < 4; ++j) p[j] = wave_sum(p[j]);
    loss_row(a_r, a_g, a_b, a_d, target_rgb[3 * n], target_rgb[3 * n + 1], target_rgb[3 * n + 2], d, rc, p, row);
    if (!FUSED && lane == 0) {
        float* out = partial + (size_t)n * 8;
#pragma unroll
        for (int j = 0; j < 7; ++j) out[j] = row[j];
        out[7] = 0.f;
    }
}

MIPSF_SINGLE_FP32 __device__ void finalize_losses(const double (&t)[9], float emd_w, uint32_t N, uint32_t S, float* __restrict__ losses,
                                const float* __restrict__ loss_weights, float* __restrict__ loss_total) {
    const double NS = (double)N * (double)S;
    float fs_w, sdf_w;
    band_weights((float)t[7], (float)t[8], fs_w, sdf_w);
    const float rgb_loss = (float)(t[0] / (3.0 * (double)N));
    const float depth_loss = (float)(t[1] / t[6]);
    float fs = (float)(t[2] / NS) * fs_w;
    float sd = (float)(t[3] / NS) * sdf_w;
// ... 446 lines not shown
    const uint32_t w = threadIdx.x / MIPSF_WAVE, lane = threadIdx.x & (MIPSF_WAVE - 1);
    const uint32_t n = blockIdx.x * PPB + w;
    if (n < N) {
        float so[3] = {0.f, 0.f, 0.f}, sd[3] = {0.f, 0.f, 0.f};
        for (uint32_t k = lane; k < S; k += MIPSF_WAVE) {
            const float z = z_vals[(size_t)n * S + k];
            const float* g = dxn + ((size_t)n * S + k) * 3;
#pragma unroll
            for (int d = 0; d < 3; ++d) {
                const float gp = (float)(((double)g[d] / nc.norm_factor) / nc.div[d]);
                so[d] += gp;
                sd[d] += gp * z;
            }
        }
#pragma unroll
        for (int d = 0; d < 3; ++d) {
            so[d] = wave_sum(so[d]);
            sd[d] = wave_sum(sd[d]);
        }
        int64_t p = owner[n];
        if (p < 0) p += P;
        if (p < 0 || p >= P) p = 0;
        const float dx = d_cam[3 * (size_t)n], dy = d_cam[3 * (size_t)n + 1], dz = d_cam[3 * (size_t)n + 2];
        if (lane < 12) {
            const int j = lane < 9 ? (int)lane / 3 : (int)lane - 9;
            const float gd = j == 0 ? sd[0] : (j == 1 ? sd[1] : sd[2]);
            const float go = j == 0 ? so[0] : (j == 1 ? so[1] : so[2]);
            const int c = (int)lane % 3;
            const float dc = c == 0 ? dx : (c == 1 ? dy : dz);
            wv[w][lane] = lane < 9 ? gd * dc : go;
        }
        if (lane == 0) wp[w] = (int)p;
    } else if (lane == 0) {
        wp[w] = -1;
    }
    __syncthreads();
    if (threadIdx.x < 12) {
        for (int ww = 0; ww < PPB; ++ww)
            if (wp[ww] >= 0) sacc[wp[ww] * 12 + (int)threadIdx.x] += wv[ww][threadIdx.x];
    }
    pose_block_finish<PPB * MIPSF_WAVE>(sacc, &is_last, P, F, K, part, ticket, rot, d_rot, d_trans, accumulate != 0);
}

static RenderCfg to_render_cfg(const mipsf_render_cfg& c) {
    RenderCfg r;
    r.trunc = c.trunc;
    r.band = (float)((double)c.sc_factor * (double)c.trunc);
    r.trunc_total = (float)((double)c.trunc * (double)c.sc_factor);
    r.depth_trunc = c.depth_trunc;
    r.rgb_missing_nonzero = c.rgb_missing_nonzero;
    r.emd_w = c.emd_w;
    return r;
}

}

using namespace mipsf;

extern "C" {

int mipsf_sample_rays(const float* rays_o, const float* rays_d, const float* target_d, const float* noise,
                      const float* z_uniform, const float* z_near_offsets, const float* z_near_nodepth,
                      const mipsf_render_cfg* cfg, float* z_vals, float* xn, uint32_t* counts, uint32_t N,
                      void* stream) {
    if (N == 0) return 0;
    MIPSF_REQUIRE(cfg && rays_o && rays_d && z_vals && xn, "null pointer");
    MIPSF_REQUIRE(z_uniform || cfg->n_uniform == 0, "null pointer: z_uniform with n_uniform = %u", cfg->n_uniform);
    const uint32_t S = cfg->n_uniform + cfg->n_near;
    MIPSF_REQUIRE(S >= 1 && S <= MAX_S, "samples per ray %u outside [1,%d]", S, MAX_S);
    MIPSF_REQUIRE(cfg->n_near == 0 || (target_d && z_near_offsets && z_near_nodepth),
                  "depth-guided samples need target_d and the near tables");
    MIPSF_REQUIRE(!cfg->perturb || noise, "perturb needs the noise tensor");
    PlaceCfg pc;
    pc.n_uniform = cfg->n_uniform;
    pc.n_near = cfg->n_near;
    pc.perturb = cfg->perturb;
    pc.trunc_total = (float)((double)cfg->trunc * (double)cfg->sc_factor);
    hipLaunchKernelGGL(sample_rays_kernel, dim3((N + RAYS_PER_BLOCK - 1) / RAYS_PER_BLOCK),
                       dim3(RAYS_PER_BLOCK * MIPSF_WAVE), 0, (hipStream_t)stream, rays_o, rays_d, target_d, noise,
                       z_uniform, z_near_offsets, z_near_nodepth, pc, make_norm(*cfg), z_vals, xn, counts, N);
    return check_launch("sample_rays");
}

int mipsf_gather_pose_place_fwd(const float* db, uint64_t n_rows, const int64_t* idx, const float* fixed_poses,
                                const float* rot, const float* trans, uint32_t F, uint32_t K, const int64_t* owner,
                                const float* noise, const float* z_uniform, const float* z_near_offsets,
                                const float* z_near_nodepth, const mipsf_render_cfg* cfg, float* d_cam, float* rgb,
                                float* depth, float* z_vals, float* xn, uint32_t* counts, uint32_t N, void* stream) {
    if (N == 0) return 0;
    MIPSF_REQUIRE(cfg && db && idx && owner && d_cam && rgb && depth && z_vals && xn, "null pointer");
    MIPSF_REQUIRE(z_uniform || cfg->n_uniform == 0, "null pointer: z_uniform with n_uniform = %u", cfg->n_uniform);
    MIPSF_REQUIRE((F == 0 || fixed_poses) && (K == 0 || (rot && trans)), "null pose pointer");
    MIPSF_REQUIRE(F + K >= 1 && F + K <= (uint32_t)PR_MAX_POSES, "number of poses %u outside [1,%d]", F + K, PR_MAX_POSES);
    const uint32_t S = cfg->n_uniform + cfg->n_near;
    MIPSF_REQUIRE(S >= 1 && S <= MAX_S, "samples per ray %u outside [1,%d]", S, MAX_S);
    MIPSF_REQUIRE(cfg->n_near == 0 || (z_near_offsets && z_near_nodepth), "depth-guided samples need the near tables");
    MIPSF_REQUIRE(!cfg->perturb || noise, "perturb needs the noise tensor");
    PlaceCfg pc;
    pc.n_uniform = cfg->n_uniform;
    pc.n_near = cfg->n_near;
    pc.perturb = cfg->perturb;
    pc.trunc_total = (float)((double)cfg->trunc * (double)cfg->sc_factor);
    hipLaunchKernelGGL(gather_pose_place_kernel, dim3((N + RAYS_PER_BLOCK - 1) / RAYS_PER_BLOCK),
                       dim3(RAYS_PER_BLOCK * MIPSF_WAVE), 0, (hipStream_t)stream, db, n_rows, idx, fixed_poses, rot, trans,
                       (int)F, (int)K, owner, noise, z_uniform, z_near_offsets, z_near_nodepth, pc, make_norm(*cfg), d_cam, rgb,
                       depth, z_vals, xn, counts, N);
    return check_launch("gather_pose_place");
}

}
namespace mipsf {
uint64_t place_pose_scratch_floats(uint32_t F, uint32_t K, uint32_t N) {
    return 1ull + 12ull * (F + K) * ((N + PPB - 1) / PPB);
}
uint64_t render_partial_floats(uint32_t N) {
    const uint64_t rows = 8ull * N, fused = 18ull * (((uint64_t)N + 15) / 16);
    return rows > fused ? rows : fused;
}
}
extern "C" {

int mipsf_place_pose_bwd(const float* dxn, const float* z_vals, const mipsf_render_cfg* cfg, const float* rot, uint32_t F,
                         uint32_t K, const int64_t* owner, const float* d_cam, float* d_rot, float* d_trans, float* scratch,
                         uint32_t N, uint32_t S, int accumulate, void* stream) {
    MIPSF_REQUIRE(K >= 1, "no optimisable pose");
    MIPSF_REQUIRE(cfg && dxn && z_vals && rot && owner && d_cam && d_rot && d_trans && scratch, "null pointer");
    MIPSF_REQUIRE(F + K <= (uint32_t)PR_MAX_POSES, "number of poses %u above %d", F + K, PR_MAX_POSES);
    if (N == 0) return 0;
    hipLaunchKernelGGL(place_pose_bwd_kernel, dim3((N + PPB - 1) / PPB), dim3(PPB * MIPSF_WAVE), 0, (hipStream_t)stream, dxn,
                       z_vals, make_norm(*cfg), d_cam, owner, rot, (int)F, (int)K, scratch + 1,
                       reinterpret_cast<uint32_t*>(scratch), d_rot, d_trans, N, S, accumulate);
    return check_launch("place_pose_bwd");
}

}

template <typename A>
static int read_args(A* a, const A* in, size_t short_size, const char* name) {
    MIPSF_REQUIRE(in != nullptr, "null argument block");
    MIPSF_REQUIRE(in->struct_size == sizeof(A) || in->struct_size == short_size, "%s: struct_size %u, this library expects %u", name,
                  in->struct_size, (unsigned)sizeof(A));
    *a = A{};
    memcpy(a, in, in->struct_size);
    return 0;
}

static int launch_render_ticket(const mipsf_render_fwd_args* a, const RenderCfg& rc, const LossFinalize& fin, const char* what,
                                hipStream_t s) {
    const uint32_t N = a->N, S = a->S;
    const dim3 grid((N + RT_RPB - 1) / RT_RPB), block(RT_RPB * MIPSF_WAVE);
    bool granted = S <= RT_MAX_S;
    if (granted) {
        const uint32_t lds = (uint32_t)RT_RPB * S * 40u;
        const int two = S > MIPSF_WAVE ? 1 : 0;
        static uint32_t attr_dev[MAX_DEVICES][2] = {};
        uint32_t& attr = attr_dev[device_slot()][a->draw ? 1 : 0];
        if (lds > 48u * 1024u && lds > attr) {
            const void* fn = a->draw ? (const void*)render_train_kernel<true, 2> : (const void*)render_train_kernel<false, 2>;
            granted = hipFuncSetAttribute(fn, hipFuncAttributeMaxDynamicSharedMemorySize, (int)lds) == hipSuccess;
            if (granted) attr = lds;
            else (void)hipGetLastError();
        }
        if (granted) {
#define RT_LAUNCH(D, K)                                                                                                              \
    hipLaunchKernelGGL((render_train_kernel<D, K>), grid, block, lds, s, a->raw, a->z_vals, a->target_rgb, a->target_d, rc, a->rgb, \
                       a->depth, a->depth_var, a->disp, a->acc, a->weights, a->partial, N, S, fin, a->draw)
            if (a->draw) { if (two) RT_LAUNCH(true, 2); else RT_LAUNCH(true, 1); }
            else { if (two) RT_LAUNCH(false, 2); else RT_LAUNCH(false, 1); }
#undef RT_LAUNCH
            return check_launch(what);
        }
        MIPSF_REQUIRE(a->draw == nullptr, "draw: this device does not grant render_train_kernel's %u bytes of LDS", lds);
    }
    hipLaunchKernelGGL((render_fwd_kernel<true, true, RT_RPB>), grid, block, 0, s, a->raw, a->z_vals, a->target_rgb, a->target_d, rc,
                       a->rgb, a->depth, a->depth_var, a->disp, a->acc, a->weights, a->partial, N, S, fin);
    return check_launch(what);
}

extern "C" {

int mipsf_render_fwd(const mipsf_render_fwd_args* a_in, void* stream) {
    mipsf_render_fwd_args block_;
    if (read_args(&block_, a_in, offsetof(mipsf_render_fwd_args, draw), "mipsf_render_fwd_args")) return 1;
    const mipsf_render_fwd_args* a = &block_;
    const uint32_t N = a->N, S = a->S;
    hipStream_t s = (hipStream_t)stream;
    if (a->sums != nullptr) {
        MIPSF_REQUIRE(a->losses == nullptr && a->loss_weights == nullptr && a->loss_total == nullptr && a->draw == nullptr,
                      "sums: the losses of a share are finished by mipsf_loss_finalize_sums, not here");
        MIPSF_REQUIRE(a->cfg && a->raw && a->z_vals && a->rgb && a->depth && a->target_rgb && a->target_d && a->counts && a->partial &&
// ... 76 lines not shown
```

### mipsfusion_amd/model/scene_rep.py

```python
import copy

import numpy as np
import os
import torch
import torch.nn as nn

from .. import ops
from .._lib import FEAT_LEVEL_MAJOR
from .decoder import MLP_reg
from .encodings import get_encoder


class _PlaceFn(torch.autograd.Function):

    @staticmethod
    def forward(ctx, rays_o, rays_d, target_d, noise, tables, rc, N, S):
        rays_o, rays_d = ops._f32c(rays_o), ops._f32c(rays_d)
        z_vals, xn, counts = ops.sample_rays(rays_o, rays_d, target_d, noise, tables, rc, N, S)
        ctx.rc, ctx.N, ctx.S = rc, N, S
        ctx.save_for_backward(z_vals)
        ctx.mark_non_differentiable(z_vals, counts)
        ctx.set_materialize_grads(False)
        return z_vals, xn, counts

    @staticmethod
    def backward(ctx, _dz, dxn, _dc):
        if dxn is None:
            return (None,) * 8
        (z_vals,) = ctx.saved_tensors
        d_o, d_d = ops.rays_bwd(ops._f32c(dxn), z_vals, ctx.rc, ctx.N, ctx.S)
        return d_o, d_d, None, None, None, None, None, None


class _NormaliseFn(torch.autograd.Function):

    @staticmethod
    def forward(ctx, pts, rc):
        ctx.rc = rc
        return ops.normalise_points(ops._f32c(pts), rc)

    @staticmethod
    def backward(ctx, dxn):
        return ops.normalise_bwd(ops._f32c(dxn), ctx.rc), None


_ROUTE_AHEAD_MIN_M = 65536
_MAX_QUERY, _QUERY_CHUNK = 1 << 24, 1 << 23


class _QueryFn(torch.autograd.Function):

    @staticmethod
    def forward(ctx, xn, owner, grid_params, *weights):
        xn = ops._f32c(xn)
        M = xn.shape[0]
        meta = owner.embed_fn.meta
        jac = None
        routed = None
        if ctx.needs_input_grad[2] and owner.route_ahead and M >= _ROUTE_AHEAD_MIN_M and not ops.resolve_deterministic(owner.deterministic):
            routed = ops.hashgrid_route_ahead(xn, meta)
        if ctx.needs_input_grad[0]:
            feat, jac = ops.hashgrid_fwd(xn, grid_params.detach(), meta, FEAT_LEVEL_MAJOR, with_jac=True)
        else:
            feat = ops.hashgrid_fwd(xn, grid_params.detach(), meta, FEAT_LEVEL_MAJOR)
        need = any(ctx.needs_input_grad)
        prec = owner.decoder_precision
        if prec == "f16" and need:
            raise RuntimeError('decoder_precision "f16" is forward-only (use "bf16x6", "f16x3" or "f32" when gradients are needed)')
        cache = owner._frozen_pack
        if cache is not None and prec in cache:
            packed, packed16 = cache[prec]
        else:
            if prec == "f32":
                packed, packed16 = ops.decoder_pack(weights), None
            else:
                packed, packed16 = None, ops.decoder_pack16(weights, precision=prec)
            if cache is not None:
                cache[prec] = (packed, packed16)
        lean = bool(need and prec in ops.SPLIT_PRECISIONS and owner.wgrad_precision in ("auto", "stream_" + prec) and owner.lean_record)
        masks_only = bool(need and prec in ops.SPLIT_PRECISIONS and not any(ctx.needs_input_grad[3:]))
        out, saved = ops.decoder_fwd(packed, feat, FEAT_LEVEL_MAJOR, xn, None, M,
                                     save="masks" if masks_only else ("lean" if lean else need), precision=prec, packed16=packed16)
        ctx.lean = lean and not masks_only
        ctx.tile_live = getattr(saved, "mipsf_tile_live", None)
        if packed is None:
            packed = packed16
        ctx.prec = prec
        if routed is not None:
            torch.cuda.current_stream(xn.device).wait_event(routed[1])
        ctx.routed = routed
        ctx.owner, ctx.M, ctx.meta, ctx.has_jac = owner, M, meta, jac is not None
        ctx.save_for_backward(xn, feat, out, saved, packed, grid_params, *weights, *([jac] if jac is not None else []))
        return out

    @staticmethod
    def backward(ctx, dout):
        xn, feat, out, saved, packed, grid_params, *weights = ctx.saved_tensors
        jac = weights.pop() if ctx.has_jac else None
        need_w = any(ctx.needs_input_grad[3:])
        need_g = ctx.needs_input_grad[2]
        need_x = ctx.needs_input_grad[0]
        if ctx.tile_live is not None:
            saved.mipsf_tile_live = ctx.tile_live
        det = ops.resolve_deterministic(ctx.owner.deterministic)
        direct = ctx.owner.accumulate_param_grads_in_place and all(
            p.is_leaf and not p._backward_hooks for p in (grid_params, *weights))
        grads = None
        if need_w:
            grads = []
            for w, need in zip(weights, ctx.needs_input_grad[3:]):
                if direct and need:
                    if w.grad is None:
                        w.grad = torch.zeros_like(w)
                    grads.append(w.grad)
                else:
                    grads.append(torch.zeros_like(w))
        dfeat, dx, _, tiles = ops.decoder_bwd(packed, feat, FEAT_LEVEL_MAJOR, xn, None, out, ops._f32c(dout), saved, grads,
                                              ctx.M, precision=ctx.prec, packed16=packed if ctx.prec != "f32" else None,
                                              wgrad_precision=("stream_" + ctx.prec) if ctx.lean else ctx.owner.wgrad_precision,
                                              recompute_h1=ctx.lean, return_tiles=True, deterministic=det)
        dparams = None
        fresh_grad = False
        if need_g:
            if direct:
                if grid_params.grad is None:
                    grid_params.grad = torch.zeros_like(grid_params)
                    fresh_grad = True
                dparams = grid_params.grad
            else:
                dparams = torch.zeros_like(grid_params)
        if need_g:
            ops.hashgrid_bwd(xn, grid_params.detach(), dfeat, dparams, ctx.meta, FEAT_LEVEL_MAJOR, None, routed=ctx.routed,
                             dparams_zero=(not direct) or fresh_grad or ctx.owner.grid_grad_is_zero_at_backward, deterministic=det)
            ctx.routed = None
        if need_x:
            ops.hashgrid_dx_from_jac(jac, dfeat, dx, ctx.meta, FEAT_LEVEL_MAJOR, tiles=tiles)
        w_out = [None] * len(weights)
        if need_w and not direct:
            w_out = [g if need else None for g, need in zip(grads, ctx.needs_input_grad[3:])]
        return (dx if need_x else None, None, None if direct else dparams, *w_out)


class _RenderFn(torch.autograd.Function):
    fuse_backward = os.environ.get("MIPSF_RENDER_FUSE_BWD", "1") != "0"

    @staticmethod
    def forward(ctx, raw, z_vals, target_rgb, target_d, counts, rc, N, S, train, loss_w=None, share_of=None):
        raw = ops._f32c(raw)
        total = None
        ctx.n_norm = None
        ctx.draw, ctx.draw_stale = None, False
        if train and share_of is not None:
            rgb, depth, var, disp, acc, _, losses, total, ctx.n_norm = ops.render_fwd(
                raw, z_vals, target_rgb, target_d, counts, rc, N, S, train, loss_weights=loss_w, share_of=share_of)
        elif train and loss_w is not None:
            if ctx.needs_input_grad[0] and S <= ops.RENDER_DRAW_MAX_S and _RenderFn.fuse_backward:
                rgb, depth, var, disp, acc, _, losses, total, ctx.draw = ops.render_fwd(
                    raw, z_vals, target_rgb, target_d, counts, rc, N, S, train, loss_weights=loss_w, want_draw=True)
            else:
                rgb, depth, var, disp, acc, _, losses, total = ops.render_fwd(raw, z_vals, target_rgb, target_d, counts, rc, N,
                                                                              S, train, loss_weights=loss_w)
        else:
            rgb, depth, var, disp, acc, _, losses = ops.render_fwd(raw, z_vals, target_rgb, target_d, counts, rc, N, S,
                                                                   train)
        ctx.rc, ctx.N, ctx.S, ctx.train = rc, N, S, train
        ctx.save_for_backward(raw, z_vals, target_rgb, target_d, counts, losses, loss_w if total is not None else None)
        ctx.mark_non_differentiable(var, disp, acc)
        ctx.set_materialize_grads(False)
        if total is not None:
            return rgb, depth, var, disp, acc, losses, total.reshape(())
        if train:
            return rgb, depth, var, disp, acc, losses
        return rgb, depth, var, disp, acc

    @staticmethod
    def backward(ctx, g_rgb, g_depth, _gv, _gd, _ga, g_losses=None, g_total=None):
        raw, z_vals, target_rgb, target_d, counts, losses, loss_w = ctx.saved_tensors
        g_rgb = ops._f32c(g_rgb) if g_rgb is not None else None
        g_depth = ops._f32c(g_depth) if g_depth is not None else None
        g_total = ops._f32c(g_total).reshape(1) if (g_total is not None and loss_w is not None) else None
        if ctx.draw is not None and not ctx.draw_stale and g_total is not None and g_losses is None and g_rgb is None and g_depth is None:
            one = ops.unit_grad(raw.device)
            if g_total.data_ptr() == one.data_ptr() and one._version == 0:
                return ctx.draw, None, None, None, None, None, None, None, None, None, None
            ctx.draw_stale = True
            draw = ops.render_bwd(raw, z_vals, target_rgb, target_d, counts, losses, ctx.rc, None, None, None, ctx.N, ctx.S,
                                  g_total=g_total, loss_weights=loss_w, keep_draw=ctx.draw)
            return draw, None, None, None, None, None, None, None, None, None, None
        if ctx.train and g_losses is None and g_total is None:
            g_losses = torch.zeros(8, dtype=torch.float32, device=raw.device)
        draw = ops.render_bwd(raw, z_vals, target_rgb, target_d, counts, losses, ctx.rc,
                              ops._f32c(g_losses) if (ctx.train and g_losses is not None) else None, g_rgb, g_depth,
                              ctx.N, ctx.S, g_total=g_total, loss_weights=loss_w, n_norm=ctx.n_norm)
        return draw, None, None, None, None, None, None, None, None, None, None


class JointEncoding(nn.Module):
    def __init__(self, config, bound_box, coords_norm_factor):
        super().__init__()
        self.config = config
        self.bounding_box = bound_box
        self.coords_norm_factor = coords_norm_factor
        self._bound64 = torch.as_tensor(bound_box).detach().to("cpu", torch.float64).tolist()
        self._half64 = torch.as_tensor(coords_norm_factor).detach().to("cpu", torch.float64).reshape(-1).tolist()
        self.accumulate_param_grads_in_place = False
        self.grid_grad_is_zero_at_backward = False
        self.deterministic = None
        self.decoder_precision = "bf16x6"
        self.wgrad_precision = "auto"
        self.lean_record = True
        self.route_ahead = False
        self.ray_share_reduce = None
        self._frozen_pack = None
        self._tables = {}
        self._jitter_ring = {}
        self.get_resolution()
        self.get_encoding(config)
        self.get_decoder(config)
        self.save_initial_param()

    def get_resolution(self):
        dim_max = max(b[1] - b[0] for b in self._bound64)
        if self.config["grid"]["voxel_sdf"] > 10:
            self.resolution_sdf = self.config["grid"]["voxel_sdf"]
        else:
            self.resolution_sdf = int(dim_max / self.config["grid"]["voxel_sdf"])

    def get_encoding(self, config):
        self.embedpos_fn, self.input_ch_pos = get_encoder(config["pos"]["enc"], n_bins=config["pos"]["n_bins"])
        self.embed_fn, self.input_ch = get_encoder(config["grid"]["enc"],
                                                   log2_hashmap_size=config["grid"]["hash_size"],
                                                   desired_resolution=256)
        if self.embed_fn.otype != "hashgrid" or self.embedpos_fn.otype != "frequency" or self.input_ch_pos != 48:
            raise ValueError("the fused HIP path is built for grid.enc=HashGrid + pos.enc=Frequency(n_bins=8), "
                             "the only combination the reference's configs use")

    def get_decoder(self, config):
        self.decoder = MLP_reg(config, input_ch=self.input_ch, input_ch_pos=self.input_ch_pos)

    def save_initial_param(self):
        self.initial_dict = copy.deepcopy(self.state_dict())

    def recover_initial_param(self):
        self.load_state_dict(self.initial_dict)

    def _rc(self, n_uniform, n_near, emd_w=0.0):
        return ops.make_render_cfg(self.config, self._bound64, self._half64, n_uniform, n_near, emd_w)

    def _linspace_tables(self, device, guided: bool):
        key = (str(device), guided)
        if key not in self._tables:
            tr, cam = self.config["training"], self.config["cam"]
            if guided:
                zu = torch.linspace(cam["near"], cam["far"], max(0, tr["n_samples_d"]))
                zoff = torch.linspace(-tr["range_d"], tr["range_d"], steps=tr["n_range_d"])
                znd = torch.linspace(cam["near"], cam["far"], steps=tr["n_range_d"])
                self._tables[key] = tuple(t.to(device=device, dtype=torch.float32).contiguous() for t in (zu, zoff, znd))
            else:
                zu = torch.linspace(cam["near"], cam["far"], tr["n_samples"]).to(device=device, dtype=torch.float32)
                self._tables[key] = (zu.contiguous(), None, None)
        return self._tables[key]

    def _query(self, x32):
        M = x32.shape[0]
        if M >= _MAX_QUERY and not (torch.is_grad_enabled() and (x32.requires_grad or any(p.requires_grad for p in self.parameters()))):
            return torch.cat([self._query(x32[i:i + _QUERY_CHUNK]) for i in range(0, M, _QUERY_CHUNK)], 0)
        return _QueryFn.apply(x32, self, self.embed_fn.params, *self.decoder.ordered_parameters())

    def __getstate__(self):
        d = self.__dict__.copy()
        d["_jitter_ring"], d["_frozen_pack"], d["ray_share_reduce"] = {}, None, None
        return d

    def __deepcopy__(self, memo):
        with torch.random.fork_rng(devices=[]):
            new = JointEncoding(self.config, self.bounding_box, self.coords_norm_factor)
        memo[id(self)] = new
        dev = self.embed_fn.params.device
        new.to(dev)
        new.load_state_dict(self.state_dict())
        new.initial_dict = copy.deepcopy(self.initial_dict)
        new.accumulate_param_grads_in_place = self.accumulate_param_grads_in_place
        new.grid_grad_is_zero_at_backward = self.grid_grad_is_zero_at_backward
        new.decoder_precision = self.decoder_precision
        new.wgrad_precision = self.wgrad_precision
        new.lean_record = self.lean_record
        new.route_ahead = self.route_ahead
        new.deterministic = self.deterministic
        new._frozen_pack = None
        new.train(self.training)
        return new

    def query_sdf(self, query_points):
        needs_grad = torch.is_grad_enabled() and (query_points.requires_grad or
                                                  any(p.requires_grad for p in self.parameters()))
        if needs_grad:
            return self.query_color_sdf(query_points)[..., 3:4]
        flat = torch.reshape(query_points, [-1, query_points.shape[-1]]) / self.config["training"]["norm_factor"]
        if not flat.is_cuda:
            raise RuntimeError("JointEncoding runs on the GPU only (no CPU fallback)")
        xn = ops._f32c(flat)
        prec = self.decoder_precision
        ws = self.decoder.ordered_parameters()
        packed = ops.decoder_pack(ws) if prec == "f32" else None
        packed16 = ops.decoder_pack16(ws, precision=prec) if prec != "f32" else None
        out = []
        for i in range(0, max(1, xn.shape[0]), _QUERY_CHUNK if xn.shape[0] >= _MAX_QUERY else max(1, xn.shape[0])):
            xc = xn[i:i + _QUERY_CHUNK] if xn.shape[0] >= _MAX_QUERY else xn
            feat = ops.hashgrid_fwd(xc, self.embed_fn.params.detach(), self.embed_fn.meta, FEAT_LEVEL_MAJOR)
            out.append(ops.decoder_fwd_sdf(packed, feat, FEAT_LEVEL_MAJOR, xc, None, xc.shape[0], precision=prec, packed16=packed16))
        return (out[0] if len(out) == 1 else torch.cat(out, 0))[:, None]

    def query_color(self, query_points):
        return torch.sigmoid(self.query_color_sdf(query_points)[..., :3])

    def query_sdf_entropy_prob(self, query_points):
        return self.query_color_sdf(query_points)[..., 3:]

    def query_color_sdf(self, query_points):
        flat = torch.reshape(query_points, [-1, query_points.shape[-1]]) / self.config["training"]["norm_factor"]
        if not flat.is_cuda:
            raise RuntimeError("JointEncoding runs on the GPU only (no CPU fallback)")
        return self._query(flat.to(torch.float32))

    def run_network(self, inputs):
        flat = torch.reshape(inputs, [-1, inputs.shape[-1]])
        if not flat.is_cuda:
            raise RuntimeError("JointEncoding runs on the GPU only (no CPU fallback)")
        rc = self._rc(1, 0)
        xn = _NormaliseFn.apply(flat, rc)
        out = self._query(xn)
        return torch.reshape(out, list(inputs.shape[:-1]) + [out.shape[-1]])

    def _render(self, rays_o, rays_d, target_rgb, target_d, noise, train, emd_w):
        if not rays_o.is_cuda:
            raise RuntimeError("JointEncoding runs on the GPU only (no CPU fallback)")
        tr = self.config["training"]
        N = rays_o.shape[0]
        guided = target_d is not None
        n_uniform = max(0, tr["n_samples_d"]) if guided else tr["n_samples"]
        n_near = tr["n_range_d"] if guided else 0
        S = n_uniform + n_near
        rc = self._rc(n_uniform, n_near, emd_w)
        if rc.perturb:
            if noise is None:
                noise = self._draw_jitter(N, S, rays_o.device)
            noise = ops._f32c(noise)
        else:
            noise = None
        tables = self._linspace_tables(rays_o.device, guided)
        td = ops._f32c(target_d).reshape(N, 1) if guided else None
        z_vals, xn, counts = _PlaceFn.apply(rays_o, rays_d, td, noise, tables, rc, N, S)
        raw = self._query(xn)
        trgb = ops._f32c(target_rgb) if train else None
        res = _RenderFn.apply(raw, z_vals, trgb, td if train else None, counts if train else None, rc, N, S, train,
                              self._objective_weights(raw.device) if train else None, self.ray_share_reduce if train else None)
        return res, z_vals, raw.reshape(N, S, 10)

    def _draw_jitter(self, N, S, device):
        from .. import hostrng
        if torch.cuda.is_current_stream_capturing():
            raise RuntimeError("JointEncoding drew its sample jitter on the host while a hipGraph was being captured: pass "
                               "`noise` (a static device tensor refilled before every replay) to forward / render_rays")
        n = N * S
        ring = self._jitter_ring.get(str(device))
        if ring is None or ring["cap"] < n:
            ring = self._jitter_ring[str(device)] = {"bufs": [torch.empty(n, dtype=torch.float32).pin_memory() for _ in range(4)],
                                                     "events": [None] * 4, "i": 0, "cap": n}
        i = ring["i"]
        ring["i"] = (i + 1) % 4
        if ring["events"][i] is not None:
            ring["events"][i].synchronize()
        buf = ring["bufs"][i][:n].view(N, S)
        with hostrng.session() as sess:
            sess.rand_(buf)
        out = buf.to(device, non_blocking=True)
        ev = torch.cuda.Event()
        ev.record(torch.cuda.current_stream(device))
        ring["events"][i] = ev
        return out

    def frozen_weights(self, begin: bool):
        self._frozen_pack = {} if begin else None

    def _objective_weights(self, device):
        tr = self.config.get("training", {})
        if not all(k in tr for k in ("rgb_weight", "depth_weight", "sdf_weight", "fs_weight")):
            return None
        vals = (float(tr["rgb_weight"]), float(tr["depth_weight"]), float(tr["sdf_weight"]), float(tr["fs_weight"]))
        key = (str(device), vals)
        if getattr(self, "_obj_w_key", None) != key:
            self._obj_w, self._obj_w_key = torch.tensor(vals, dtype=torch.float32, device=device), key
        return self._obj_w

    def forward_from_table(self, table, rows, rot, trans, fixed_poses, owner, noise, EMD_w=0.01, accumulate_in_place=False):
        if not self.training:
            raise RuntimeError("forward_from_table is the training branch (use forward / render_rays for evaluation)")
        tr = self.config["training"]
        n_uniform, n_near = max(0, tr["n_samples_d"]), tr["n_range_d"]
        S, N = n_uniform + n_near, rows.shape[0]
        rc = self._rc(n_uniform, n_near, float(EMD_w))
        if rc.perturb and noise is None:
            raise ValueError("forward_from_table needs the jitter noise as a device tensor")
        tables = self._linspace_tables(table.device, True)
        trgb, td, z_vals, xn, counts = ops.GatherPosePlaceFn.apply(rot, trans, fixed_poses, owner, table, rows,
                                                                   ops._f32c(noise) if rc.perturb else None, tables, rc, S,
                                                                   accumulate_in_place)
        raw = self._query(xn)
        res = _RenderFn.apply(raw, z_vals, trgb, td, counts, rc, N, S, True, self._objective_weights(raw.device),
                              self.ray_share_reduce)
        rgb, depth, losses = res[0], res[1], res[5]
        ret = {"rgb": rgb, "depth": depth, "rgb_loss": losses[0], "depth_loss": losses[1], "sdf_loss": losses[2],
               "fs_loss": losses[3], "psnr": losses[4:5].detach(), "_loss_vec": losses}
        if len(res) > 6:
            ret["_loss_total"], ret["_loss_total_weights"] = res[6], self._obj_w_key[1]
        return ret

    def render_rays(self, rays_o, rays_d, target_d=None, noise=None):
        (rgb, depth, var, disp, acc), z_vals, raw = self._render(rays_o, rays_d, None, target_d, noise, False, 0.0)
        return {"rgb": rgb, "depth": depth, "disp_map": disp, "acc_map": acc, "depth_var": var, "z_vals": z_vals,
                "raw": raw}

    def forward(self, rays_o, rays_d, target_rgb, target_d, EMD_w=0.01, noise=None):
        if not self.training:
            return self.render_rays(rays_o, rays_d, target_d=target_d, noise=noise)
        res, _z, _raw = self._render(rays_o, rays_d, target_rgb, target_d, noise, True, float(EMD_w))
        rgb, depth, losses = res[0], res[1], res[5]
        total = res[6] if len(res) > 6 else None
        ret = {"rgb": rgb, "depth": depth, "rgb_loss": losses[0], "depth_loss": losses[1], "sdf_loss": losses[2],
               "fs_loss": losses[3], "psnr": losses[4:5].detach(), "_loss_vec": losses}
        if total is not None:
            ret["_loss_total"], ret["_loss_total_weights"] = total, self._obj_w_key[1]
        return ret
```

### mipsfusion_amd/ops.py

```python
from __future__ import annotations

import ctypes as C
import os
from typing import Optional

import torch

from . import _lib
from ._lib import FEAT_AOS, FEAT_LEVEL_MAJOR, check, dptr, lib, stream_ptr

DECODER_PARAM_ORDER = ("pts_linear.0.weight", "pts_linear.0.bias", "pts_linear.2.weight", "pts_linear.2.bias",
                       "rgb_linear.0.weight", "rgb_linear.0.bias", "sdf_linear.0.weight", "sdf_linear.0.bias",
                       "sdf_linear.2.weight", "sdf_linear.2.bias")
_DEC_FIELDS = ("w_pts0", "b_pts0", "w_pts2", "b_pts2", "w_rgb0", "b_rgb0", "w_sdf0", "b_sdf0", "w_sdf2", "b_sdf2")
_DEC_SHAPES = ((128, 51), (128,), (128, 128), (128,), (3, 115), (3,), (128, 96), (128,), (5, 128), (5,))


PROFILE = None


class _timed:
    def __init__(self, name, stream=None):
        self.name, self.stream = name, stream

    def __enter__(self):
        if PROFILE is not None:
            self.a = torch.cuda.Event(enable_timing=True)
            self.b = torch.cuda.Event(enable_timing=True)
            self.a.record(self.stream)

    def __exit__(self, *exc):
        if PROFILE is not None:
            self.b.record(self.stream)
            PROFILE.setdefault(self.name, []).append((self.a, self.b))


def profile_summary():
    out = {}
    for k, pairs in (PROFILE or {}).items():
        ms = [a.elapsed_time(b) for a, b in pairs]
        out[k] = (len(ms), sum(ms) / max(1, len(ms)))
    return out


def _f32c(t: torch.Tensor) -> torch.Tensor:
    if t.dtype != torch.float32:
        t = t.to(torch.float32)
    return t.contiguous()


def hashgrid_fwd(x: torch.Tensor, params: torch.Tensor, meta, layout=FEAT_AOS, with_jac: bool = False):
    M = x.shape[0]
    nf = meta.n_levels * meta.n_features
    out = torch.empty((M, nf) if layout == FEAT_AOS else (meta.n_levels, M, meta.n_features),
                      dtype=torch.float32, device=x.device)
    if with_jac:
        jac = torch.empty((meta.n_levels, 3, M, 2), dtype=torch.float32, device=x.device)
        with _timed("hashgrid_fwd"):
            check(lib().mipsf_hashgrid_fwd(dptr(x), dptr(params), dptr(out), dptr(jac), M, C.byref(meta), layout,
                                           stream_ptr()), "hashgrid_fwd (with the Jacobian)")
        return out, jac
    with _timed("hashgrid_fwd"):
        check(lib().mipsf_hashgrid_fwd(dptr(x), dptr(params), dptr(out), None, M, C.byref(meta), layout, stream_ptr()),
              "hashgrid_fwd")
    return out


class LiveList:
    __slots__ = ("buf",)

    def __init__(self, buf):
        self.buf = buf


def hashgrid_dx_from_jac(jac, dout, dx, meta, layout=FEAT_AOS, tiles=None):
    M = dx.shape[0]
    if isinstance(tiles, LiveList):
        with _timed("hashgrid_dx"):
            check(lib().mipsf_hashgrid_dx_from_jac_list(dptr(jac), dptr(dout), dptr(dx), dptr(tiles.buf, torch.int32), M,
                                                        C.byref(meta), layout, stream_ptr()), "hashgrid_dx_from_jac_list")
        return
    with _timed("hashgrid_dx"):
        check(lib().mipsf_hashgrid_dx_from_jac(dptr(jac), dptr(dout), dptr(dx), dptr(tiles, torch.int32), M,
                                               C.byref(meta), layout, stream_ptr()), "hashgrid_dx_from_jac")


_SIDE_STREAMS = {}
SKIP_ZERO_TILES = os.environ.get("MIPSF_NO_TILE_SKIP", "0") != "1"
_LAST_TILE_LIVE = None
COMPACT_LIVE = os.environ.get("MIPSF_NO_COMPACT", "0") != "1"


def last_live_tile_share() -> Optional[float]:
    if _LAST_TILE_LIVE is None:
        return None
    buf, M, compacted = _LAST_TILE_LIVE
    if compacted:
        return float(buf[1].item()) / max(1, (M + 31) // 32)
    counts = buf[32:512:64].cpu()
    return float(counts.sum().item()) / max(1, (M + 31) // 32)


_LAST_SCATTER_DOUT = None


def last_live_record_share() -> Optional[float]:
    if _LAST_SCATTER_DOUT is None:
        return None
    d = _LAST_SCATTER_DOUT.reshape(-1, 2)
    return float(((d[:, 0] != 0) | (d[:, 1] != 0)).float().mean().item())


def side_stream(device) -> "torch.cuda.Stream":
    key = torch.device(device).index if torch.device(device).index is not None else torch.cuda.current_device()
    if key not in _SIDE_STREAMS:
        _SIDE_STREAMS[key] = torch.cuda.Stream(device=key)
    return _SIDE_STREAMS[key]


def hashgrid_route_ahead(x, meta):
    M = x.shape[0]
    n = _lib.buffer_size(_lib.SIZE_HASHGRID_BWD_SCRATCH, M, 0, 0, meta)
    scratch = torch.empty(n, dtype=torch.float32, device=x.device)
    main, side = torch.cuda.current_stream(x.device), side_stream(x.device)
    side.wait_stream(main)
    with _timed("hashgrid_route", side):
        check(lib().mipsf_hashgrid_route(dptr(x), dptr(scratch), M, C.byref(meta), C.c_void_p(side.cuda_stream)),
              "hashgrid_route")
    ev = torch.cuda.Event()
    ev.record(side)
    return scratch, ev


_ZEROED = {}
_lib.KEPT_BLOCK_CACHES.append(_ZEROED)


def _zeroed_words(device, n, tag):
    key = (device.index, stream_ptr(), tag, n)
    buf = _ZEROED.get(key)
    if buf is None:
        buf = _ZEROED[key] = torch.zeros(n, dtype=torch.int32, device=device)
    return buf


_SCATTER_COUNTERS = {}
_lib.KEPT_BLOCK_CACHES.append(_SCATTER_COUNTERS)


def _scatter_counters(device, meta):
    n = _lib.buffer_size(_lib.SIZE_HASHGRID_COUNTER_WORDS, meta=meta)
    key = (device.index, stream_ptr(), n)
    buf = _SCATTER_COUNTERS.get(key)
    if buf is None:
        buf = _SCATTER_COUNTERS[key] = torch.zeros(n, dtype=torch.int32, device=device)
    return buf


LEAN_DACT = not bool(os.environ.get("MIPSF_FULL_DACT"))
# ... 476 lines not shown
        fixed = _f32c(fixed) if fixed is not None and fixed.numel() else None
        owner = owner.to(torch.int64).contiguous()
        F = 0 if fixed is None else fixed.shape[0]
        K = rot.shape[0]
        dev = rot.device
        if table is not None:
            flat = table.reshape(-1, 7)
            N = rows.shape[0]
            d_cam = torch.empty((N, 3), dtype=torch.float32, device=dev)
            rgb = torch.empty((N, 3), dtype=torch.float32, device=dev)
            depth = torch.empty((N, 1), dtype=torch.float32, device=dev)
        else:
            d_cam = _f32c(d_cam)
            N = d_cam.shape[0]
        rays_o = torch.empty((N, 3), dtype=torch.float32, device=dev)
        rays_d = torch.empty((N, 3), dtype=torch.float32, device=dev)
        with _timed("pose_rays_fwd"):
            if table is not None:
                check(lib().mipsf_pose_rays_fwd(dptr(flat), flat.shape[0], dptr(rows, torch.int64), dptr(fixed),
                                                dptr(rot), dptr(trans), F, K, dptr(owner, torch.int64), dptr(d_cam),
                                                dptr(rgb), dptr(depth), dptr(rays_o), dptr(rays_d), N, stream_ptr()),
                      "pose_rays_fwd (rows of the ray table)")
            else:
                check(lib().mipsf_pose_rays_fwd(None, 0, None, dptr(fixed), dptr(rot), dptr(trans), F, K,
                                                dptr(owner, torch.int64), dptr(d_cam), None, None, dptr(rays_o), dptr(rays_d), N,
                                                stream_ptr()), "pose_rays_fwd")
        ctx.F, ctx.K, ctx.N = F, K, N
        ctx.save_for_backward(rot, owner, d_cam)
        ctx.set_materialize_grads(False)
        if table is not None:
            ctx.mark_non_differentiable(rgb, depth)
            return rays_o, rays_d, rgb, depth
        return rays_o, rays_d

    @staticmethod
    def backward(ctx, g_o, g_d, _g_rgb=None, _g_depth=None):
        rot, owner, d_cam = ctx.saved_tensors
        scratch = _pose_scratch(rot.device, ctx.F, ctx.K, ctx.N)
        g_o = _f32c(g_o) if g_o is not None else None
        g_d = _f32c(g_d) if g_d is not None else None
        direct = ctx.params is not None and all(
            p.is_leaf and p.requires_grad and not p._backward_hooks and p.dtype == torch.float32 and p.is_contiguous()
            for p in ctx.params)
        if direct:
            for p in ctx.params:
                if p.grad is None:
                    p.grad = torch.zeros_like(p)
            d_rot, d_trans = ctx.params[0].grad, ctx.params[1].grad
        else:
            d_rot = torch.empty((ctx.K, 4), dtype=torch.float32, device=rot.device)
            d_trans = torch.empty((ctx.K, 3), dtype=torch.float32, device=rot.device)
        with _timed("pose_rays_bwd"):
            check(lib().mipsf_pose_rays_bwd(dptr(g_o), dptr(g_d), dptr(rot), ctx.F, ctx.K, dptr(owner, torch.int64),
                                            dptr(d_cam), dptr(d_rot), dptr(d_trans), dptr(scratch), ctx.N,
                                            1 if direct else 0, stream_ptr()), "pose_rays_bwd")
        if direct:
            return None, None, None, None, None, None, None, None
        return d_rot, d_trans, None, None, None, None, None, None


def pose_rays(rot, trans, fixed_poses, owner, d_cam, accumulate_in_place=False):
    return PoseRaysFn.apply(rot, trans, fixed_poses, owner, d_cam, accumulate_in_place)


def gather_pose_rays(table, rows, rot, trans, fixed_poses, owner, accumulate_in_place=False):
    return PoseRaysFn.apply(rot, trans, fixed_poses, owner, None, accumulate_in_place, table, rows.to(torch.int64).contiguous())


class GatherPosePlaceFn(torch.autograd.Function):

    @staticmethod
    def forward(ctx, rot, trans, fixed, owner, table, rows, noise, tables, rc, S, in_place):
        ctx.params = (rot, trans) if in_place else None
        rot, trans = _f32c(rot), _f32c(trans)
        fixed = _f32c(fixed) if fixed is not None and fixed.numel() else None
        owner = owner.to(torch.int64).contiguous()
        rows = rows.to(torch.int64).contiguous()
        F = 0 if fixed is None else fixed.shape[0]
        K, N, dev = rot.shape[0], rows.shape[0], rot.device
        flat = table.reshape(-1, 7)
        e = lambda *sh: torch.empty(sh, dtype=torch.float32, device=dev)
        d_cam, rgb, depth, z_vals, xn = e(N, 3), e(N, 3), e(N, 1), e(N, S), e(N * S, 3)
        counts = torch.empty((N, 2), dtype=torch.int32, device=dev)
        zu, zoff, znd = tables
        with _timed("sample_rays"):
            check(lib().mipsf_gather_pose_place_fwd(dptr(flat), flat.shape[0], dptr(rows, torch.int64), dptr(fixed), dptr(rot),
                                                    dptr(trans), F, K, dptr(owner, torch.int64), dptr(noise), dptr(zu),
                                                    dptr(zoff), dptr(znd), C.byref(rc), dptr(d_cam), dptr(rgb), dptr(depth),
                                                    dptr(z_vals), dptr(xn), dptr(counts, torch.int32), N, stream_ptr()),
                  "gather_pose_place_fwd")
        ctx.F, ctx.K, ctx.N, ctx.S, ctx.rc = F, K, N, S, rc
        ctx.save_for_backward(rot, owner, d_cam, z_vals)
        ctx.mark_non_differentiable(rgb, depth, z_vals, counts)
        ctx.set_materialize_grads(False)
        return rgb, depth, z_vals, xn, counts

    @staticmethod
    def backward(ctx, _g_rgb, _g_depth, _g_z, dxn, _g_counts):
        if dxn is None:
            return (None,) * 11
        rot, owner, d_cam, z_vals = ctx.saved_tensors
        n = _lib.buffer_size(_lib.SIZE_PLACE_POSE_SCRATCH, ctx.N, ctx.F, ctx.K)
        key = (rot.device.index, stream_ptr(), "place", n)
        scratch = _POSE_SCRATCH.get(key)
        if scratch is None:
            scratch = _POSE_SCRATCH[key] = torch.zeros(n, dtype=torch.float32, device=rot.device)
        direct = ctx.params is not None and all(
            p.is_leaf and p.requires_grad and not p._backward_hooks and p.dtype == torch.float32 and p.is_contiguous()
            for p in ctx.params)
        if direct:
            for p in ctx.params:
                if p.grad is None:
                    p.grad = torch.zeros_like(p)
            d_rot, d_trans = ctx.params[0].grad, ctx.params[1].grad
        else:
            d_rot = torch.empty((ctx.K, 4), dtype=torch.float32, device=rot.device)
            d_trans = torch.empty((ctx.K, 3), dtype=torch.float32, device=rot.device)
        with _timed("rays_bwd"):
            check(lib().mipsf_place_pose_bwd(dptr(_f32c(dxn)), dptr(z_vals), C.byref(ctx.rc), dptr(rot), ctx.F, ctx.K,
                                             dptr(owner, torch.int64), dptr(d_cam), dptr(d_rot), dptr(d_trans), dptr(scratch),
                                             ctx.N, ctx.S, 1 if direct else 0, stream_ptr()), "place_pose_bwd")
        if direct:
            return (None,) * 11
        return (d_rot, d_trans) + (None,) * 9


def adam_advance(step_dev, hyper_dev, lr, beta1, beta2):
    adam_advance_n([(step_dev, hyper_dev, lr, beta1, beta2)])


def adam_advance_n(groups):
    n = len(groups)
    steps = (C.c_void_p * n)(*[dptr(g[0], torch.int32) for g in groups])
    hypers = (C.c_void_p * n)(*[dptr(g[1]) for g in groups])
    lr = (C.c_float * n)(*[g[2] for g in groups])
    b1 = (C.c_float * n)(*[g[3] for g in groups])
    b2 = (C.c_float * n)(*[g[4] for g in groups])
    check(lib().mipsf_adam_advance_n(steps, hypers, lr, b1, b2, n, stream_ptr()), "adam_advance_n")


def adam_step(param, grad, exp_avg, exp_avg_sq, lr, beta1, beta2, eps, weight_decay, step, zero_grad=False,
              hyper_dev=None):
    with _timed("adam_step" if param.numel() > (1 << 20) else "adam_step_small"):
        check(lib().mipsf_adam_step(dptr(param), dptr(grad), dptr(exp_avg), dptr(exp_avg_sq), param.numel(), lr,
                                    beta1, beta2, eps, weight_decay, step, dptr(hyper_dev),
                                    1 if zero_grad else 0, stream_ptr()), "adam_step")


def adam_step_multi(params, grads, exp_avgs, exp_avg_sqs, lr, beta1, beta2, eps, weight_decay, step, zero_grad=False,
                    hyper_dev=None):
    for i in range(0, len(params), _lib.ADAM_MAX_TENSORS):
        chunk = slice(i, i + _lib.ADAM_MAX_TENSORS)
        t = _lib.AdamTensors()
        t.count = len(params[chunk])
        for j, (p, g, m, v) in enumerate(zip(params[chunk], grads[chunk], exp_avgs[chunk], exp_avg_sqs[chunk])):
            t.param[j], t.grad[j], t.exp_avg[j], t.exp_avg_sq[j] = dptr(p), dptr(g), dptr(m), dptr(v)
            t.numel[j] = p.numel()
        with _timed("adam_step_small"):
            check(lib().mipsf_adam_step_multi(C.byref(t), lr, beta1, beta2, eps, weight_decay, step,
                                              dptr(hyper_dev), 1 if zero_grad else 0, stream_ptr()),
                  "adam_step_multi")


def adam_step_small(groups, zero_grad=False):
    d = _lib.AdamSmall()
    d.n_groups = len(groups)
    ti = 0
    for gi, (step_dev, hyper_dev, lr, b1, b2, eps, wd, tensors) in enumerate(groups):
        d.step_dev[gi], d.hyper_dev[gi] = dptr(step_dev, torch.int32), dptr(hyper_dev)
        d.lr[gi], d.beta1[gi], d.beta2[gi], d.eps[gi], d.weight_decay[gi] = lr, b1, b2, eps, wd
        for p, g, m, v in tensors:
            d.param[ti], d.grad[ti], d.exp_avg[ti], d.exp_avg_sq[ti] = dptr(p), dptr(g), dptr(m), dptr(v)
            d.numel[ti], d.group_of[ti] = p.numel(), gi
            ti += 1
    d.n_tensors = ti
    with _timed("adam_step_small"):
        check(lib().mipsf_adam_step_small(C.byref(d), 1 if zero_grad else 0, stream_ptr()), "adam_step_small")


def adam_step_all(groups, ticket, zero_grad=False):
    d = _lib.AdamSmall()
# ... 63 lines not shown
```

Baseline: 442.0 million rays*samples/s.

## Skip hash-grid Jacobian and dx for fixed-pose rays; fold scatter partials in-kernel

The ray gather/placement kernel now emits a per-ray flag that says whether that ray's pose is being optimised. The flag is passed through the query into the hash-grid forward, which then skips writing Jacobian entries for rays whose pose is fixed, and into the dx kernel, which writes zeros for those rays instead of reducing over levels. Separately, the backward scatter gains an arrival counter per bin, so the last block to finish a bin folds the partial slices itself instead of leaving that to a separate fold pass. This relies on agent-scope atomics and fences, and the flag-gated path adds extra API entry points and argument plumbing.

```diff
diff --git a/include/mipsf_compact.h b/include/mipsf_compact.h
--- a/include/mipsf_compact.h
+++ b/include/mipsf_compact.h
@@ -15,6 +15,18 @@
 int mipsf_hashgrid_dx_from_jac_list(const float* jac, const float* dout, float* dx, const uint32_t* live_list, uint32_t M,
                                     const mipsf_grid_meta* meta_host, int layout, void* stream);
 
+int mipsf_gather_pose_place_fwd_masked(const float* db, uint64_t n_rows, const int64_t* idx, const float* fixed_poses,
+                                       const float* rot, const float* trans, uint32_t F, uint32_t K, const int64_t* owner,
+                                       const float* noise, const float* z_uniform, const float* z_near_offsets,
+                                       const float* z_near_nodepth, const mipsf_render_cfg* cfg_host, float* d_cam, float* rgb,
+                                       float* depth, float* z_vals, float* xn, uint32_t* counts, uint32_t* wants_dx, uint32_t N,
+                                       void* stream);
+int mipsf_hashgrid_fwd_masked(const float* x, const float* params, float* out, float* jac, const uint32_t* ray_mask, uint32_t S,
+                              uint32_t M, const mipsf_grid_meta* meta_host, int layout, void* stream);
+int mipsf_hashgrid_dx_from_jac_masked(const float* jac, const float* dout, float* dx, const uint32_t* tile_live,
+                                      const uint32_t* live_list, const uint32_t* ray_mask, uint32_t S, uint32_t M,
+                                      const mipsf_grid_meta* meta_host, int layout, void* stream);
+
 #ifdef __cplusplus
 }
 #endif
diff --git a/mipsfusion_amd/_lib.py b/mipsfusion_amd/_lib.py
--- a/mipsfusion_amd/_lib.py
+++ b/mipsfusion_amd/_lib.py
@@ -123,8 +123,7 @@
     "mipsf_hashgrid_fwd": (_I, [_P, _P, _P, _P, _U32, C.POINTER(GridMeta), _I, _P]),
     "mipsf_hashgrid_dx_from_jac": (_I, [_P, _P, _P, _P, _U32, C.POINTER(GridMeta), _I, _P]),
     "mipsf_hashgrid_bwd": (_I, [C.POINTER(HashgridBwdArgs), _P]),
-    "mipsf_hashgrid_route": (_I, [_P, _P, _U32, C.POINTER(GridMeta), _P]),
-    "mipsf_hashgrid_indices": (_I, [_P, _P, _U32, C.POINTER(GridMeta), _P]),
+    "mipsf_hashgrid_route": (_I, [_P, _P, _U32, C.POINTER(GridMeta), _P]),    "mipsf_hashgrid_indices": (_I, [_P, _P, _U32, C.POINTER(GridMeta), _P]),
     "mipsf_freq_fwd": (_I, [_P, _P, _U32, _U32, _U32, _P]),
     "mipsf_freq_bwd": (_I, [_P, _P, _P, _U32, _U32, _U32, _P]),
     "mipsf_decoder_pack": (_I, [C.POINTER(DecoderWeights), _P, _P]),
@@ -175,6 +174,10 @@
 COMPACT_SIGNATURES = {
     "mipsf_decoder_live_compact": (_I, [_P, _U32, _P, _P, _P, _I, _P]),
     "mipsf_hashgrid_dx_from_jac_list": (_I, [_P, _P, _P, _P, _U32, C.POINTER(GridMeta), _I, _P]),
+    "mipsf_gather_pose_place_fwd_masked": (_I, [_P, _U64, _P, _P, _P, _P, _U32, _U32, _P, _P, _P, _P, _P, C.POINTER(RenderCfg),
+                                                _P, _P, _P, _P, _P, _P, _P, _U32, _P]),
+    "mipsf_hashgrid_fwd_masked": (_I, [_P, _P, _P, _P, _P, _U32, _U32, C.POINTER(GridMeta), _I, _P]),
+    "mipsf_hashgrid_dx_from_jac_masked": (_I, [_P, _P, _P, _P, _P, _P, _U32, _U32, C.POINTER(GridMeta), _I, _P]),
 }
 
 MESH_SIGNATURES = {
@@ -410,6 +413,13 @@
     return int(v)
 
 
+def hashgrid_counter_layout(meta) -> dict:
+    end = buffer_size(SIZE_HASHGRID_COUNTER_WORDS, meta=meta)
+    bins = (end - 4) // 4
+    return {"count": 0, "nitems": bins, "arrive": bins + 4, "first": 2 * bins + 4, "parts": 3 * bins + 4, "end": end,
+            "n_bins": bins}
+
+
 _lib: Optional[C.CDLL] = None
 
 
diff --git a/mipsfusion_amd/csrc/hashgrid.hip b/mipsfusion_amd/csrc/hashgrid.hip
--- a/mipsfusion_amd/csrc/hashgrid.hip
+++ b/mipsfusion_amd/csrc/hashgrid.hip
@@ -113,11 +113,16 @@
     }
 }
 
+__device__ __forceinline__ bool ray_wants_dx(const uint32_t* __restrict__ ray_mask, uint32_t S, uint32_t i) {
+    return ray_mask == nullptr || ray_mask[S == 64u ? i >> 6 : i / S] != 0u;
+}
+
 template <int LAYOUT, bool JAC>
 __global__ __launch_bounds__(HG_BLOCK) void hashgrid_fwd_kernel(const float* __restrict__ x,
                                                                 const float2* __restrict__ table,
                                                                 float* __restrict__ out, float* __restrict__ jac,
-                                                                uint32_t M, GridLevels g, uint32_t nchunk) {
+                                                                uint32_t M, GridLevels g, uint32_t nchunk,
+                                                                const uint32_t* __restrict__ ray_mask, uint32_t S) {
     uint32_t chunk;
     const int level = decode_level(g.n_levels, nchunk, chunk);
     if (level >= (int)g.n_levels) return;
@@ -145,7 +150,7 @@
     typedef float f32x2_t __attribute__((ext_vector_type(2)));
     f32x2_t* dst = reinterpret_cast<f32x2_t*>(out + feat_index<LAYOUT>(i, level, M, g.n_levels));
     __builtin_nontemporal_store(f32x2_t{a0, a1}, dst);
-    if (JAC) {
+    if (JAC && ray_wants_dx(ray_mask, S, i)) {
         f32x2_t* j2 = reinterpret_cast<f32x2_t*>(jac) + (size_t)level * 3 * M + i;
 #pragma unroll
         for (int d = 0; d < 3; ++d) {
@@ -214,7 +219,8 @@
     uint32_t max_slice;
     uint32_t dense_bins;
     uint32_t fresh;
-    uint32_t w_count, w_first, w_parts, w_nitems, w_items;
+    uint32_t fold_launch;
+    uint32_t w_count, w_arrive, w_first, w_parts, w_nitems, w_items;
     uint64_t w_records, w_partial, w_end;
 };
 
@@ -244,6 +250,7 @@
     uint64_t w = 0;
     p.w_count = (uint32_t)w, w += bins;
     p.w_nitems = (uint32_t)w, w += 4;
+    p.w_arrive = (uint32_t)w, w += bins;
     p.w_first = (uint32_t)w, w += bins;
     p.w_parts = (uint32_t)w, w += bins;
     w = (w + 3) / 4 * 4;
@@ -584,10 +591,41 @@
     return bin < plan.dense_bins ? SC_PART_DENSE : SC_PART;
 }
 
+#ifndef MIPSF_SC_PUBLISH_WT
+#define MIPSF_SC_PUBLISH_WT 1
+#endif
+
+template <bool AGENT>
+__device__ __forceinline__ float2 fold_entry(const float2* p2, uint32_t parts, float2 cur) {
+    float2 a = make_float2(0.f, 0.f);
+    for (uint32_t q = 0; q < parts; q += 8) {
+        float2 v[8];
+#pragma unroll
+        for (uint32_t k = 0; k < 8; ++k) {
+            v[k] = make_float2(0.f, 0.f);
+            if (q + k < parts) {
+                if (AGENT) {
+                    const unsigned long long u = __hip_atomic_load(
+                        reinterpret_cast<const unsigned long long*>(p2 + (size_t)(q + k) * SC_MAX_SLICE), __ATOMIC_RELAXED,
+                        __HIP_MEMORY_SCOPE_AGENT);
+                    v[k] = make_float2(__uint_as_float((uint32_t)u), __uint_as_float((uint32_t)(u >> 32)));
+                } else {
+                    v[k] = p2[(size_t)(q + k) * SC_MAX_SLICE];
+                }
+            }
+        }
+#pragma unroll
+        for (uint32_t k = 0; k < 8; ++k) a.x += v[k].x, a.y += v[k].y;
+    }
+    cur.x += a.x, cur.y += a.y;
+    return cur;
+}
+
 template <int LAYOUT>
 __device__ __forceinline__ void scatter_item(const float* __restrict__ x, const float* __restrict__ dout,
                                              float* __restrict__ dparams, uint32_t M, const GridLevels& g,
-                                             const ScatterPlan& plan, uint32_t* __restrict__ ws, double* __restrict__ acc,
+                                             const ScatterPlan& plan, uint32_t* __restrict__ ws, uint32_t* __restrict__ cw,
+                                             uint32_t* sh_flag, double* __restrict__ acc,
                                              const uint4 desc, const uint32_t item_index) {
     const uint32_t item = desc.x;
     const uint32_t sc_plane1 = plan.max_slice;
@@ -824,12 +862,46 @@
             }
         }
     } else {
-        float2* pdst = reinterpret_cast<float2*>(reinterpret_cast<float*>(ws) + plan.w_partial) +
-                       (size_t)item_index * SC_MAX_SLICE;
+        float2* part0 = reinterpret_cast<float2*>(reinterpret_cast<float*>(ws) + plan.w_partial);
+        float2* pdst = part0 + (size_t)item_index * SC_MAX_SLICE;
+        if (plan.fold_launch) {
+            for (uint32_t e = threadIdx.x; e < count; e += SC_BLOCK) {
+                const double2 a = a2(e);
+                pdst[e] = make_float2((float)a.x, (float)a.y);
+            }
+            return;
+        }
         for (uint32_t e = threadIdx.x; e < count; e += SC_BLOCK) {
             const double2 a = a2(e);
+#if MIPSF_SC_PUBLISH_WT
+            __hip_atomic_store(reinterpret_cast<unsigned long long*>(pdst + e),
+                               (unsigned long long)__float_as_uint((float)a.x) | ((unsigned long long)__float_as_uint((float)a.y) << 32),
+                               __ATOMIC_RELAXED, __HIP_MEMORY_SCOPE_AGENT);
+#else
             pdst[e] = make_float2((float)a.x, (float)a.y);
-        }
+#endif
+        }
+        asm volatile("s_waitcnt vmcnt(0)" ::: "memory");
+        __syncthreads();
+        if (threadIdx.x == 0) {
+#if !MIPSF_SC_PUBLISH_WT
+            __builtin_amdgcn_fence(__ATOMIC_RELEASE, "agent");
+            asm volatile("s_waitcnt vmcnt(0)" ::: "memory");
+#endif
+            const uint32_t before = __hip_atomic_fetch_add(&cw[plan.w_arrive + bin], 1u, __ATOMIC_RELAXED, __HIP_MEMORY_SCOPE_AGENT);
+            const bool last = before == desc.z - 1u;
+            if (last) {
+                __builtin_amdgcn_fence(__ATOMIC_ACQUIRE, "agent");
+                asm volatile("s_waitcnt vmcnt(0)" ::: "memory");
+            }
+            *sh_flag = last ? 1u : 0u;
+        }
+        __syncthreads();
+        if (*sh_flag == 0u) return;
+        const float2* p2 = part0 + (size_t)(item_index - part) * SC_MAX_SLICE;
+        for (uint32_t e = threadIdx.x; e < count; e += SC_BLOCK)
+            dst[e] = fold_entry<true>(p2 + e, desc.z, plan.fresh ? make_float2(0.f, 0.f) : dst[e]);
+        if (threadIdx.x == 0) __hip_atomic_store(&cw[plan.w_arrive + bin], 0u, __ATOMIC_RELAXED, __HIP_MEMORY_SCOPE_AGENT);
     }
 }
 
@@ -910,7 +982,7 @@
 #ifdef MIPSF_SC_TRACE
         const uint64_t tr_t0 = wall_clock64();
 #endif
-        scatter_item<LAYOUT>(x, dout, dparams, M, g, plan, ws, acc, desc, i);
+        scatter_item<LAYOUT>(x, dout, dparams, M, g, plan, ws, cw, &wtot[0], acc, desc, i);
 #ifdef MIPSF_SC_TRACE
         __syncthreads();
         if (t == 0) {
@@ -949,17 +1021,7 @@
     const float2* p2 = reinterpret_cast<const float2*>(reinterpret_cast<const float*>(ws) + plan.w_partial) +
                        (size_t)cw[plan.w_first + bin] * SC_MAX_SLICE + e;
     float2* d = reinterpret_cast<float2*>(dparams) + g.offsets[level] + begin + e;
-    float2 cur = plan.fresh ? make_float2(0.f, 0.f) : *d;
-    float2 a = make_float2(0.f, 0.f);
-    for (uint32_t q = 0; q < parts; q += 8) {
-        float2 v[8];
-#pragma unroll
-        for (uint32_t k = 0; k < 8; ++k) v[k] = q + k < parts ? p2[(size_t)(q + k) * SC_MAX_SLICE] : make_float2(0.f, 0.f);
-#pragma unroll
-        for (uint32_t k = 0; k < 8; ++k) a.x += v[k].x, a.y += v[k].y;
-    }
-    cur.x += a.x, cur.y += a.y;
-    *d = cur;
+    *d = fold_entry<false>(p2, parts, plan.fresh ? make_float2(0.f, 0.f) : *d);
 }
 
 template <int LAYOUT>
@@ -1010,7 +1072,8 @@
                                                               const float* __restrict__ dout, float* __restrict__ dx,
                                                               uint32_t M, uint32_t L,
                                                               const uint32_t* __restrict__ tiles,
-                                                              const uint32_t* __restrict__ live_list) {
+                                                              const uint32_t* __restrict__ live_list,
+                                                              const uint32_t* __restrict__ ray_mask, uint32_t S) {
     uint32_t i = blockIdx.x * blockDim.x + threadIdx.x;
     if (live_list != nullptr) {
         if (i >= M || i >= live_list[0]) return;
@@ -1029,6 +1092,10 @@
         i = tiles[mipsf::dl::TL_HEADER + q * cap + (k - first)] * 32u + (i & 31u);
     }
     if (i >= M) return;
+    if (!ray_wants_dx(ray_mask, S, i)) {
+        dx[3 * (size_t)i] = 0.f, dx[3 * (size_t)i + 1] = 0.f, dx[3 * (size_t)i + 2] = 0.f;
+        return;
+    }
     float a[3] = {0.f, 0.f, 0.f};
     for (uint32_t l = 0; l < L; ++l) {
         const float2* j2 = reinterpret_cast<const float2*>(jac) + (size_t)l * 3 * M + i;
@@ -1387,18 +1454,25 @@
 
 extern "C" {
 
+static int check_ray_mask(const uint32_t* ray_mask, uint32_t S, uint32_t M) {
+    MIPSF_REQUIRE(ray_mask == nullptr || (S >= 1 && M % S == 0), "ray mask: %u samples are not whole rays of %u", M, S);
+    return 0;
+}
+
 static int hashgrid_fwd_impl(const float* x, const float* params, float* out, float* jac, uint32_t M,
-                             const mipsf_grid_meta* meta, int layout, void* stream) {
+                             const mipsf_grid_meta* meta, int layout, void* stream, const uint32_t* ray_mask = nullptr,
+                             uint32_t S = 0) {
     GridLevels g;
     if (int rc = to_levels(meta, g)) return rc;
     if (M == 0) return 0;
     MIPSF_REQUIRE(x && params && out, "null pointer");
     MIPSF_REQUIRE(layout == MIPSF_FEAT_AOS || layout == MIPSF_FEAT_LEVEL_MAJOR, "bad layout %d", layout);
+    if (int rc = check_ray_mask(ray_mask, S, M)) return rc;
     uint32_t nchunk;
     const uint32_t nb = grid_blocks(M, g.n_levels, nchunk);
     hipStream_t s = (hipStream_t)stream;
     const float2* table = reinterpret_cast<const float2*>(params);
-#define FWD(LAY, J) hipLaunchKernelGGL((hashgrid_fwd_kernel<LAY, J>), dim3(nb), dim3(HG_BLOCK), 0, s, x, table, out, jac, M, g, nchunk)
+#define FWD(LAY, J) hipLaunchKernelGGL((hashgrid_fwd_kernel<LAY, J>), dim3(nb), dim3(HG_BLOCK), 0, s, x, table, out, jac, M, g, nchunk, ray_mask, S)
     if (layout == MIPSF_FEAT_AOS) { if (jac) FWD(MIPSF_FEAT_AOS, true); else FWD(MIPSF_FEAT_AOS, false); }
     else { if (jac) FWD(MIPSF_FEAT_LEVEL_MAJOR, true); else FWD(MIPSF_FEAT_LEVEL_MAJOR, false); }
 #undef FWD
@@ -1409,20 +1483,31 @@
                        const mipsf_grid_meta* meta, int layout, void* stream) {
     return hashgrid_fwd_impl(x, params, out, jac, M, meta, layout, stream);
 }
+int mipsf_hashgrid_fwd_masked(const float* x, const float* params, float* out, float* jac, const uint32_t* ray_mask, uint32_t S,
+                              uint32_t M, const mipsf_grid_meta* meta, int layout, void* stream) {
+    return hashgrid_fwd_impl(x, params, out, jac, M, meta, layout, stream, ray_mask, S);
+}
 
 static int dx_from_jac(const float* jac, const float* dout, float* dx, const uint32_t* tile_live, const uint32_t* live_list, uint32_t M,
-                       const mipsf_grid_meta* meta, int layout, void* stream) {
+                       const mipsf_grid_meta* meta, int layout, void* stream, const uint32_t* ray_mask = nullptr, uint32_t S = 0) {
     GridLevels g;
     if (int rc = to_levels(meta, g)) return rc;
     if (M == 0) return 0;
     MIPSF_REQUIRE(jac && dout && dx, "null pointer");
     MIPSF_REQUIRE(layout == MIPSF_FEAT_AOS || layout == MIPSF_FEAT_LEVEL_MAJOR, "bad layout %d", layout);
+    MIPSF_REQUIRE(!(tile_live && live_list), "tile_live and live_list are alternatives");
+    if (int rc = check_ray_mask(ray_mask, S, M)) return rc;
     hipStream_t s = (hipStream_t)stream;
     if (layout == MIPSF_FEAT_AOS)
-        hipLaunchKernelGGL(hashgrid_dx_jac_kernel<MIPSF_FEAT_AOS>, dim3((M + 255) / 256), dim3(256), 0, s, jac, dout, dx, M, g.n_levels, tile_live, live_list);
+        hipLaunchKernelGGL(hashgrid_dx_jac_kernel<MIPSF_FEAT_AOS>, dim3((M + 255) / 256), dim3(256), 0, s, jac, dout, dx, M, g.n_levels, tile_live, live_list, ray_mask, S);
     else
-        hipLaunchKernelGGL(hashgrid_dx_jac_kernel<MIPSF_FEAT_LEVEL_MAJOR>, dim3((M + 255) / 256), dim3(256), 0, s, jac, dout, dx, M, g.n_levels, tile_live, live_list);
+        hipLaunchKernelGGL(hashgrid_dx_jac_kernel<MIPSF_FEAT_LEVEL_MAJOR>, dim3((M + 255) / 256), dim3(256), 0, s, jac, dout, dx, M, g.n_levels, tile_live, live_list, ray_mask, S);
     return check_launch("hashgrid_dx_from_jac");
+}
+int mipsf_hashgrid_dx_from_jac_masked(const float* jac, const float* dout, float* dx, const uint32_t* tile_live,
+                                      const uint32_t* live_list, const uint32_t* ray_mask, uint32_t S, uint32_t M,
+                                      const mipsf_grid_meta* meta, int layout, void* stream) {
+    return dx_from_jac(jac, dout, dx, tile_live, live_list, M, meta, layout, stream, ray_mask, S);
 }
 int mipsf_hashgrid_dx_from_jac(const float* jac, const float* dout, float* dx, const uint32_t* tile_live, uint32_t M,
                                const mipsf_grid_meta* meta, int layout, void* stream) {
@@ -1455,6 +1540,7 @@
 }
 }
 extern "C" {
+
 
 #ifdef MIPSF_SC_TRACE
 uint64_t mipsf_hashgrid_trace_words(const mipsf_grid_meta* meta, uint32_t M, uint32_t* n_rows, uint32_t* bin0) {
@@ -1490,7 +1576,7 @@
 static int launch_route(const float* x, const float* dout, int layout, uint32_t* ws, uint32_t* cw, bool clear, uint32_t M,
                         const GridLevels& g, const ScatterPlan& plan, hipStream_t s) {
     if (clear) {
-        const uint32_t nz = plan.w_nitems + 4;
+        const uint32_t nz = plan.w_first;
         hipLaunchKernelGGL(scatter_zero_kernel, dim3((nz + 255) / 256), dim3(256), 0, s, cw, nz);
     }
     const uint32_t rb = route_groups(g.n_levels) * ((M + RT_BLOCK * SC_ROUTE_UNR - 1) / (RT_BLOCK * SC_ROUTE_UNR));
@@ -1524,6 +1610,10 @@
     hipStream_t s = (hipStream_t)stream;
     ScatterPlan plan = make_plan(g, M);
     plan.fresh = fresh ? 1u : 0u;
+    {
+        const char* e = getenv("MIPSF_SC_FOLD_LAUNCH");
+        plan.fold_launch = (e && e[0] && e[0] != '0') ? 1u : 0u;
+    }
     if (int rc = check_plan(plan, g, M)) return rc;
     uint32_t* ws = reinterpret_cast<uint32_t*>(scratch);
     uint32_t* cw = counters ? counters : ws;
@@ -1556,9 +1646,11 @@
         if (layout == MIPSF_FEAT_AOS) SCATTER(MIPSF_FEAT_AOS); else SCATTER(MIPSF_FEAT_LEVEL_MAJOR);
 #undef SCATTER
         if (int e = check_launch("hashgrid_scatter")) return e;
-        hipLaunchKernelGGL(hashgrid_scatter_reduce_kernel, dim3(plan.n_bins, (plan.max_slice + 255) / 256), dim3(256), 0, s,
-                           dparams, g, plan, ws, cw);
-        if (int e = check_launch("hashgrid_scatter_reduce")) return e;
+        if (plan.fold_launch) {
+            hipLaunchKernelGGL(hashgrid_scatter_reduce_kernel, dim3(plan.n_bins, (plan.max_slice + 255) / 256), dim3(256), 0, s,
+                               dparams, g, plan, ws, cw);
+            if (int e = check_launch("hashgrid_scatter_reduce")) return e;
+        }
     }
     if (dx) {
         uint32_t nchunk;
diff --git a/mipsfusion_amd/csrc/render.hip b/mipsfusion_amd/csrc/render.hip
--- a/mipsfusion_amd/csrc/render.hip
+++ b/mipsfusion_amd/csrc/render.hip
@@ -108,7 +108,7 @@
     const float* __restrict__ noise, const float* __restrict__ z_uniform, const float* __restrict__ z_near_off,
     const float* __restrict__ z_near_nodepth, PlaceCfg pc, NormCfg nc, float* __restrict__ d_cam, float* __restrict__ rgb,
     float* __restrict__ depth, float* __restrict__ z_vals, float* __restrict__ xn, uint32_t* __restrict__ counts,
-    uint32_t N) {
+    uint32_t* __restrict__ wants_dx, uint32_t N) {
     __shared__ float zs[RAYS_PER_BLOCK][MAX_S];
     __shared__ float sb[RAYS_PER_BLOCK][MAX_S];
     __shared__ float sa[MAX_S];
@@ -132,6 +132,7 @@
     int64_t p = owner[n];
     if (p < 0) p += F + K;
     const bool in_range = p >= 0 && p < F + K;
+    if (wants_dx != nullptr && lane == 0) wants_dx[n] = (in_range ? (int)p : 0) >= F ? 1u : 0u;
     const Mat34 m = load_pose(fixed, rot, trans, F, in_range ? (int)p : 0);
     const float dx = in_range ? v[0] : __builtin_nanf(""), dy = v[1], dz = v[2];
     float o[3], dv[3];
@@ -744,11 +745,12 @@
     return check_launch("sample_rays");
 }
 
-int mipsf_gather_pose_place_fwd(const float* db, uint64_t n_rows, const int64_t* idx, const float* fixed_poses,
-                                const float* rot, const float* trans, uint32_t F, uint32_t K, const int64_t* owner,
-                                const float* noise, const float* z_uniform, const float* z_near_offsets,
-                                const float* z_near_nodepth, const mipsf_render_cfg* cfg, float* d_cam, float* rgb,
-                                float* depth, float* z_vals, float* xn, uint32_t* counts, uint32_t N, void* stream) {
+static int gather_pose_place_fwd(const float* db, uint64_t n_rows, const int64_t* idx, const float* fixed_poses,
+                                 const float* rot, const float* trans, uint32_t F, uint32_t K, const int64_t* owner,
+                                 const float* noise, const float* z_uniform, const float* z_near_offsets,
+                                 const float* z_near_nodepth, const mipsf_render_cfg* cfg, float* d_cam, float* rgb,
+                                 float* depth, float* z_vals, float* xn, uint32_t* counts, uint32_t* wants_dx, uint32_t N,
+                                 void* stream) {
     if (N == 0) return 0;
     MIPSF_REQUIRE(cfg && db && idx && owner && d_cam && rgb && depth && z_vals && xn, "null pointer");
     MIPSF_REQUIRE(z_uniform || cfg->n_uniform == 0, "null pointer: z_uniform with n_uniform = %u", cfg->n_uniform);
@@ -766,8 +768,27 @@
     hipLaunchKernelGGL(gather_pose_place_kernel, dim3((N + RAYS_PER_BLOCK - 1) / RAYS_PER_BLOCK),
                        dim3(RAYS_PER_BLOCK * MIPSF_WAVE), 0, (hipStream_t)stream, db, n_rows, idx, fixed_poses, rot, trans,
                        (int)F, (int)K, owner, noise, z_uniform, z_near_offsets, z_near_nodepth, pc, make_norm(*cfg), d_cam, rgb,
-                       depth, z_vals, xn, counts, N);
+                       depth, z_vals, xn, counts, wants_dx, N);
     return check_launch("gather_pose_place");
+}
+
+int mipsf_gather_pose_place_fwd(const float* db, uint64_t n_rows, const int64_t* idx, const float* fixed_poses,
+                                const float* rot, const float* trans, uint32_t F, uint32_t K, const int64_t* owner,
+                                const float* noise, const float* z_uniform, const float* z_near_offsets,
+                                const float* z_near_nodepth, const mipsf_render_cfg* cfg, float* d_cam, float* rgb,
+                                float* depth, float* z_vals, float* xn, uint32_t* counts, uint32_t N, void* stream) {
+    return gather_pose_place_fwd(db, n_rows, idx, fixed_poses, rot, trans, F, K, owner, noise, z_uniform, z_near_offsets,
+                                 z_near_nodepth, cfg, d_cam, rgb, depth, z_vals, xn, counts, nullptr, N, stream);
+}
+int mipsf_gather_pose_place_fwd_masked(const float* db, uint64_t n_rows, const int64_t* idx, const float* fixed_poses,
+                                       const float* rot, const float* trans, uint32_t F, uint32_t K, const int64_t* owner,
+                                       const float* noise, const float* z_uniform, const float* z_near_offsets,
+                                       const float* z_near_nodepth, const mipsf_render_cfg* cfg, float* d_cam, float* rgb,
+                                       float* depth, float* z_vals, float* xn, uint32_t* counts, uint32_t* wants_dx, uint32_t N,
+                                       void* stream) {
+    MIPSF_REQUIRE(wants_dx != nullptr || N == 0, "null wants_dx");
+    return gather_pose_place_fwd(db, n_rows, idx, fixed_poses, rot, trans, F, K, owner, noise, z_uniform, z_near_offsets,
+                                 z_near_nodepth, cfg, d_cam, rgb, depth, z_vals, xn, counts, wants_dx, N, stream);
 }
 
 }
diff --git a/mipsfusion_amd/model/scene_rep.py b/mipsfusion_amd/model/scene_rep.py
--- a/mipsfusion_amd/model/scene_rep.py
+++ b/mipsfusion_amd/model/scene_rep.py
@@ -51,7 +51,7 @@
 class _QueryFn(torch.autograd.Function):
 
     @staticmethod
-    def forward(ctx, xn, owner, grid_params, *weights):
+    def forward(ctx, xn, owner, grid_params, ray_mask, *weights):
         xn = ops._f32c(xn)
         M = xn.shape[0]
         meta = owner.embed_fn.meta
@@ -60,7 +60,7 @@
         if ctx.needs_input_grad[2] and owner.route_ahead and M >= _ROUTE_AHEAD_MIN_M and not ops.resolve_deterministic(owner.deterministic):
             routed = ops.hashgrid_route_ahead(xn, meta)
         if ctx.needs_input_grad[0]:
-            feat, jac = ops.hashgrid_fwd(xn, grid_params.detach(), meta, FEAT_LEVEL_MAJOR, with_jac=True)
+            feat, jac = ops.hashgrid_fwd(xn, grid_params.detach(), meta, FEAT_LEVEL_MAJOR, with_jac=True, ray_mask=ray_mask)
         else:
             feat = ops.hashgrid_fwd(xn, grid_params.detach(), meta, FEAT_LEVEL_MAJOR)
         need = any(ctx.needs_input_grad)
@@ -78,7 +78,7 @@
             if cache is not None:
                 cache[prec] = (packed, packed16)
         lean = bool(need and prec in ops.SPLIT_PRECISIONS and owner.wgrad_precision in ("auto", "stream_" + prec) and owner.lean_record)
-        masks_only = bool(need and prec in ops.SPLIT_PRECISIONS and not any(ctx.needs_input_grad[3:]))
+        masks_only = bool(need and prec in ops.SPLIT_PRECISIONS and not any(ctx.needs_input_grad[4:]))
         out, saved = ops.decoder_fwd(packed, feat, FEAT_LEVEL_MAJOR, xn, None, M,
                                      save="masks" if masks_only else ("lean" if lean else need), precision=prec, packed16=packed16)
         ctx.lean = lean and not masks_only
@@ -90,6 +90,7 @@
             torch.cuda.current_stream(xn.device).wait_event(routed[1])
         ctx.routed = routed
         ctx.owner, ctx.M, ctx.meta, ctx.has_jac = owner, M, meta, jac is not None
+        ctx.ray_mask = ray_mask if jac is not None else None
         ctx.save_for_backward(xn, feat, out, saved, packed, grid_params, *weights, *([jac] if jac is not None else []))
         return out
 
@@ -97,7 +98,7 @@
     def backward(ctx, dout):
         xn, feat, out, saved, packed, grid_params, *weights = ctx.saved_tensors
         jac = weights.pop() if ctx.has_jac else None
-        need_w = any(ctx.needs_input_grad[3:])
+        need_w = any(ctx.needs_input_grad[4:])
         need_g = ctx.needs_input_grad[2]
         need_x = ctx.needs_input_grad[0]
         if ctx.tile_live is not None:
@@ -108,7 +109,7 @@
         grads = None
         if need_w:
             grads = []
-            for w, need in zip(weights, ctx.needs_input_grad[3:]):
+            for w, need in zip(weights, ctx.needs_input_grad[4:]):
                 if direct and need:
                     if w.grad is None:
                         w.grad = torch.zeros_like(w)
@@ -134,11 +135,12 @@
                              dparams_zero=(not direct) or fresh_grad or ctx.owner.grid_grad_is_zero_at_backward, deterministic=det)
             ctx.routed = None
         if need_x:
-            ops.hashgrid_dx_from_jac(jac, dfeat, dx, ctx.meta, FEAT_LEVEL_MAJOR, tiles=tiles)
+            ops.hashgrid_dx_from_jac(jac, dfeat, dx, ctx.meta, FEAT_LEVEL_MAJOR, tiles=tiles,
+                                     ray_mask=ctx.ray_mask)
         w_out = [None] * len(weights)
         if need_w and not direct:
-            w_out = [g if need else None for g, need in zip(grads, ctx.needs_input_grad[3:])]
-        return (dx if need_x else None, None, None if direct else dparams, *w_out)
+            w_out = [g if need else None for g, need in zip(grads, ctx.needs_input_grad[4:])]
+        return (dx if need_x else None, None, None if direct else dparams, None, *w_out)
 
 
 class _RenderFn(torch.autograd.Function):
@@ -210,6 +212,7 @@
         self.wgrad_precision = "auto"
         self.lean_record = True
         self.route_ahead = False
+        self.mask_fixed_rays = os.environ.get("MIPSF_NO_DX_MASK", "0") != "1"
         self.ray_share_reduce = None
         self._frozen_pack = None
         self._tables = {}
@@ -261,11 +264,11 @@
                 self._tables[key] = (zu.contiguous(), None, None)
         return self._tables[key]
 
-    def _query(self, x32):
+    def _query(self, x32, ray_mask=None):
         M = x32.shape[0]
         if M >= _MAX_QUERY and not (torch.is_grad_enabled() and (x32.requires_grad or any(p.requires_grad for p in self.parameters()))):
             return torch.cat([self._query(x32[i:i + _QUERY_CHUNK]) for i in range(0, M, _QUERY_CHUNK)], 0)
-        return _QueryFn.apply(x32, self, self.embed_fn.params, *self.decoder.ordered_parameters())
+        return _QueryFn.apply(x32, self, self.embed_fn.params, ray_mask, *self.decoder.ordered_parameters())
 
     def __getstate__(self):
         d = self.__dict__.copy()
@@ -286,6 +289,7 @@
         new.wgrad_precision = self.wgrad_precision
         new.lean_record = self.lean_record
         new.route_ahead = self.route_ahead
+        new.mask_fixed_rays = self.mask_fixed_rays
         new.deterministic = self.deterministic
         new._frozen_pack = None
         new.train(self.training)
@@ -403,10 +407,10 @@
         if rc.perturb and noise is None:
             raise ValueError("forward_from_table needs the jitter noise as a device tensor")
         tables = self._linspace_tables(table.device, True)
-        trgb, td, z_vals, xn, counts = ops.GatherPosePlaceFn.apply(rot, trans, fixed_poses, owner, table, rows,
-                                                                   ops._f32c(noise) if rc.perturb else None, tables, rc, S,
-                                                                   accumulate_in_place)
-        raw = self._query(xn)
+        trgb, td, z_vals, xn, counts, wants_dx = ops.GatherPosePlaceFn.apply(rot, trans, fixed_poses, owner, table, rows,
+                                                                             ops._f32c(noise) if rc.perturb else None, tables,
+                                                                             rc, S, accumulate_in_place)
+        raw = self._query(xn, wants_dx if self.mask_fixed_rays else None)
         res = _RenderFn.apply(raw, z_vals, trgb, td, counts, rc, N, S, True, self._objective_weights(raw.device),
                               self.ray_share_reduce)
         rgb, depth, losses = res[0], res[1], res[5]
diff --git a/mipsfusion_amd/ops.py b/mipsfusion_amd/ops.py
--- a/mipsfusion_amd/ops.py
+++ b/mipsfusion_amd/ops.py
@@ -49,16 +49,23 @@
     return t.contiguous()
 
 
-def hashgrid_fwd(x: torch.Tensor, params: torch.Tensor, meta, layout=FEAT_AOS, with_jac: bool = False):
+def hashgrid_fwd(x: torch.Tensor, params: torch.Tensor, meta, layout=FEAT_AOS, with_jac: bool = False, ray_mask=None):
     M = x.shape[0]
     nf = meta.n_levels * meta.n_features
     out = torch.empty((M, nf) if layout == FEAT_AOS else (meta.n_levels, M, meta.n_features),
                       dtype=torch.float32, device=x.device)
     if with_jac:
         jac = torch.empty((meta.n_levels, 3, M, 2), dtype=torch.float32, device=x.device)
+        if ray_mask is not None and (ray_mask.shape[0] == 0 or M % ray_mask.shape[0] != 0):
+            raise RuntimeError(f"ray mask: {M} samples are not whole rays of {ray_mask.shape[0]} rays")
         with _timed("hashgrid_fwd"):
-            check(lib().mipsf_hashgrid_fwd(dptr(x), dptr(params), dptr(out), dptr(jac), M, C.byref(meta), layout,
-                                           stream_ptr()), "hashgrid_fwd (with the Jacobian)")
+            if ray_mask is not None:
+                check(lib().mipsf_hashgrid_fwd_masked(dptr(x), dptr(params), dptr(out), dptr(jac), dptr(ray_mask, torch.int32),
+                                                      M // ray_mask.shape[0], M, C.byref(meta), layout, stream_ptr()),
+                      "hashgrid_fwd (with the Jacobian, masked)")
+            else:
+                check(lib().mipsf_hashgrid_fwd(dptr(x), dptr(params), dptr(out), dptr(jac), M, C.byref(meta), layout,
+                                               stream_ptr()), "hashgrid_fwd (with the Jacobian)")
         return out, jac
     with _timed("hashgrid_fwd"):
         check(lib().mipsf_hashgrid_fwd(dptr(x), dptr(params), dptr(out), None, M, C.byref(meta), layout, stream_ptr()),
@@ -73,8 +80,19 @@
         self.buf = buf
 
 
-def hashgrid_dx_from_jac(jac, dout, dx, meta, layout=FEAT_AOS, tiles=None):
+def hashgrid_dx_from_jac(jac, dout, dx, meta, layout=FEAT_AOS, tiles=None, ray_mask=None):
     M = dx.shape[0]
+    if ray_mask is not None:
+        if ray_mask.shape[0] == 0 or M % ray_mask.shape[0] != 0:
+            raise RuntimeError(f"ray mask: {M} samples are not whole rays of {ray_mask.shape[0]} rays")
+        lst = isinstance(tiles, LiveList)
+        with _timed("hashgrid_dx"):
+            check(lib().mipsf_hashgrid_dx_from_jac_masked(dptr(jac), dptr(dout), dptr(dx),
+                                                          None if lst else dptr(tiles, torch.int32),
+                                                          dptr(tiles.buf, torch.int32) if lst else None,
+                                                          dptr(ray_mask, torch.int32), M // ray_mask.shape[0], M,
+                                                          C.byref(meta), layout, stream_ptr()), "hashgrid_dx_from_jac_masked")
+        return
     if isinstance(tiles, LiveList):
         with _timed("hashgrid_dx"):
             check(lib().mipsf_hashgrid_dx_from_jac_list(dptr(jac), dptr(dout), dptr(dx), dptr(tiles.buf, torch.int32), M,
@@ -717,21 +735,23 @@
         e = lambda *sh: torch.empty(sh, dtype=torch.float32, device=dev)
         d_cam, rgb, depth, z_vals, xn = e(N, 3), e(N, 3), e(N, 1), e(N, S), e(N * S, 3)
         counts = torch.empty((N, 2), dtype=torch.int32, device=dev)
+        wants_dx = torch.empty((N,), dtype=torch.int32, device=dev)
         zu, zoff, znd = tables
         with _timed("sample_rays"):
-            check(lib().mipsf_gather_pose_place_fwd(dptr(flat), flat.shape[0], dptr(rows, torch.int64), dptr(fixed), dptr(rot),
-                                                    dptr(trans), F, K, dptr(owner, torch.int64), dptr(noise), dptr(zu),
-                                                    dptr(zoff), dptr(znd), C.byref(rc), dptr(d_cam), dptr(rgb), dptr(depth),
-                                                    dptr(z_vals), dptr(xn), dptr(counts, torch.int32), N, stream_ptr()),
+            check(lib().mipsf_gather_pose_place_fwd_masked(dptr(flat), flat.shape[0], dptr(rows, torch.int64), dptr(fixed),
+                                                           dptr(rot), dptr(trans), F, K, dptr(owner, torch.int64), dptr(noise),
+                                                           dptr(zu), dptr(zoff), dptr(znd), C.byref(rc), dptr(d_cam), dptr(rgb),
+                                                           dptr(depth), dptr(z_vals), dptr(xn), dptr(counts, torch.int32),
+                                                           dptr(wants_dx, torch.int32), N, stream_ptr()),
                   "gather_pose_place_fwd")
         ctx.F, ctx.K, ctx.N, ctx.S, ctx.rc = F, K, N, S, rc
         ctx.save_for_backward(rot, owner, d_cam, z_vals)
-        ctx.mark_non_differentiable(rgb, depth, z_vals, counts)
+        ctx.mark_non_differentiable(rgb, depth, z_vals, counts, wants_dx)
         ctx.set_materialize_grads(False)
-        return rgb, depth, z_vals, xn, counts
-
-    @staticmethod
-    def backward(ctx, _g_rgb, _g_depth, _g_z, dxn, _g_counts):
+        return rgb, depth, z_vals, xn, counts, wants_dx
+
+    @staticmethod
+    def backward(ctx, _g_rgb, _g_depth, _g_z, dxn, _g_counts, _g_wants):
         if dxn is None:
             return (None,) * 11
         rot, owner, d_cam, z_vals = ctx.saved_tensors
```

Measured after the change: 449.6 million rays*samples/s (median of 6 runs). 1.02x the previous value.
